# continental/uncertainty-detection-autolabeling

Measured on AMD Instinct MI355X. Metric: images*MC-samples/sec, EfficientDet-D0 MC-dropout serve (preprocess+net xT+decode+NMS), higher is better.
Workload: dtype f32 (tensors and accumulators float32; 1x1 products on the matrix cores as two fp16 pieces per operand, 3 cross terms (~2^-22 per product; float32-class, the default))

## Files before the change

### include/uda_hip.h

```cpp
#ifndef UDA_HIP_H_
#define UDA_HIP_H_

#include <stdint.h>

#ifdef __cplusplus
extern "C" {
#endif

#define UDA_ABI_VERSION 5
#define UDA_MAX_LEVELS 8
#define UDA_MAX_FUSE_INPUTS 3

typedef struct uda_buf_desc {
  int32_t H, W, C;
  int32_t per_sample;
  int64_t offset;
  int32_t kind;
  int32_t level;
} uda_buf_desc_t;

enum uda_op_kind {
  UDA_OP_STEM = 1,
  UDA_OP_PW = 2,
  UDA_OP_DW = 3,
  UDA_OP_SE = 4,
  UDA_OP_FUSE = 5,
  UDA_OP_POOL = 6,
  UDA_OP_MBX = 7,
  UDA_OP_SEP = 8
};
enum uda_act { UDA_ACT_NONE = 0, UDA_ACT_SWISH = 1, UDA_ACT_RELU = 2, UDA_ACT_RELU6 = 3, UDA_ACT_HSWISH = 4, UDA_ACT_MISH = 5 };
enum uda_resample { UDA_RS_NONE = 0, UDA_RS_NEAREST_UP = 1, UDA_RS_MAXPOOL = 2 };

typedef struct uda_op {
  int32_t kind;
  int32_t in[UDA_MAX_FUSE_INPUTS];
  int32_t out;
  int32_t se_scale;
  int32_t se_partial;
  int32_t residual;
  int32_t k, stride;
  int32_t act;
  int64_t w_off;
  int64_t bias_off;
  int64_t bn_scale_off;
  int64_t bn_shift_off;
  int64_t se_w1_off, se_b1_off, se_w2_off, se_b2_off;
  int32_t se_mid;
  int32_t drop_site;
  int32_t resample[UDA_MAX_FUSE_INPUTS];
  float fuse_w[UDA_MAX_FUSE_INPUTS];
  int32_t n_in;
  int32_t drop_site2;
  int64_t w2_off;
  int64_t bn2_scale_off, bn2_shift_off;
  int32_t launch_group;
  int32_t fuse_in;
  int32_t fuse_act;
} uda_op_t;

typedef struct uda_drop_site {
  int32_t channels;
  float rate;
} uda_drop_site_t;

enum uda_decode { UDA_DECODE_PLAIN = 0, UDA_DECODE_LNORM = 1, UDA_DECODE_FALSEDEC = 2,
                  UDA_DECODE_SAMPLE = 3  };
enum uda_post_mode { UDA_POST_GLOBAL = 0, UDA_POST_PER_CLASS = 1 };
enum uda_pw_scheme {
  UDA_SPLIT_NONE = 0,
  UDA_SPLIT_BF16X2 = 2,
  UDA_SPLIT_BF16X3 = 3,
  UDA_SPLIT_F16X2 = 4,
  UDA_SPLIT_F16X1 = 5
};

typedef struct uda_model {
  int32_t abi_version;
  int32_t image_h, image_w;
  float mean_rgb[3], stddev_rgb[3];
  int32_t num_levels;
  int32_t level_h[UDA_MAX_LEVELS], level_w[UDA_MAX_LEVELS];
  int32_t anchors_per_loc;
  int32_t num_classes;
  int32_t loss_attenuation;
  int32_t mc_samples;
  int32_t cls_stacked, box_stacked;
  int32_t has_uncert;
  int32_t decode_method;
  int32_t enable_softmax;
  float nms_soft_sigma;
  float nms_iou_thresh, nms_score_thresh;
  int32_t max_output_size;
  int32_t max_nms_inputs;
  int32_t post_mode;
  int32_t chunk_images;
  int32_t max_images;
  int64_t arena_floats;
  int32_t n_drop_sites;
  int32_t decode_nsamples;
  int32_t pw_scheme;
} uda_model_t;

typedef struct uda_ctx uda_ctx_t;

int uda_create(const uda_model_t* model, const uda_buf_desc_t* bufs, int32_t n_bufs,
               const uda_op_t* ops, int32_t n_ops, const uda_drop_site_t* sites,
               const float* weights, int64_t n_weights, const float* anchors ,
               int32_t device, uda_ctx_t** out);
void uda_destroy(uda_ctx_t* ctx);
const char* uda_last_error(const uda_ctx_t* ctx);

uint32_t uda_crc32c(const void* data, uint64_t n, uint32_t crc);

int uda_set_images_u8(uda_ctx_t* ctx, const uint8_t* images, int32_t n, int32_t h, int32_t w);
int uda_set_images_u8_ragged(uda_ctx_t* ctx, const uint8_t* const* images, int32_t n, const int32_t* h, const int32_t* w);
int uda_prefetch_images_u8(uda_ctx_t* ctx, const uint8_t* images, int32_t n, int32_t h, int32_t w);
int uda_prefetch_images_u8_ragged(uda_ctx_t* ctx, const uint8_t* const* images, int32_t n, const int32_t* h, const int32_t* w);
int uda_swap_prefetched(uda_ctx_t* ctx);
int uda_set_images_u8_device(uda_ctx_t* ctx, const void* images_dev, int32_t n, int32_t h, int32_t w);
int uda_input_u8_device(uda_ctx_t* ctx, const void** images_dev, int32_t* n, int32_t* h, int32_t* w);
int uda_set_images_f32(uda_ctx_t* ctx, const float* images, int32_t n, const float* image_scales);

int uda_set_dropout_seed(uda_ctx_t* ctx, uint64_t seed);
int uda_set_dropout_image_offset(uda_ctx_t* ctx, int64_t first_image);
int uda_set_dropout_sample_shard(uda_ctx_t* ctx, int32_t t_first, int32_t t_stride, int32_t t_total);
int uda_set_dropout_masks(uda_ctx_t* ctx, const float* masks, int64_t n_floats);
int uda_get_dropout_masks(uda_ctx_t* ctx, float* masks, int64_t n_floats);

int uda_run(uda_ctx_t* ctx, int32_t post_mode, int32_t run_post);
int uda_synchronize(uda_ctx_t* ctx);
int uda_run_async(uda_ctx_t* ctx, int32_t post_mode, int32_t* ticket);
int uda_run_consistency(uda_ctx_t* ctx, int32_t post_mode);
int uda_get_consistency(uda_ctx_t* ctx, double* iou, uint8_t* agree);
int uda_get_augmented_u8(uda_ctx_t* ctx, uint8_t* out, int64_t n_bytes);
int uda_collect(uda_ctx_t* ctx, int32_t ticket, float* boxes, float* scores, float* classes, int32_t* valid, float* logits);
int uda_collect_device(uda_ctx_t* ctx, int32_t ticket, int32_t rows, int32_t with_logits, void** dev_ptr, int32_t* cols);
int uda_drain(uda_ctx_t* ctx);
int64_t uda_range_demotions(const uda_ctx_t* ctx);
int uda_debug_op_scheme(const uda_ctx_t* ctx, int32_t op, int32_t* scheme, float* w_scale, float* a_scale, int32_t* out_f16);
int64_t uda_nms_prefix_fallbacks(const uda_ctx_t* ctx);
// ... 194 lines not shown
```

### uncertainty-detection-autolabeling_amd/capi.py

```python
import ctypes as C
import os
import subprocess

HERE = os.path.dirname(os.path.abspath(__file__))
CSRC = os.path.join(HERE, "csrc")
LIB_PATH = os.environ.get("UDA_LIB") or os.path.join(CSRC, "libuda_hip.so")
HEADER = os.path.join(os.path.dirname(HERE), "include", "uda_hip.h")

UDA_ABI_VERSION = 5
MAX_LEVELS = 8
MAX_FUSE = 3

OP_STEM, OP_PW, OP_DW, OP_SE, OP_FUSE, OP_POOL, OP_MBX, OP_SEP = 1, 2, 3, 4, 5, 6, 7, 8
ACT_NONE, ACT_SWISH, ACT_RELU, ACT_RELU6, ACT_HSWISH, ACT_MISH = 0, 1, 2, 3, 4, 5
RS_NONE, RS_NEAREST_UP, RS_MAXPOOL = 0, 1, 2
DECODE_PLAIN, DECODE_LNORM, DECODE_FALSEDEC, DECODE_SAMPLE = 0, 1, 2, 3
POST_GLOBAL, POST_PER_CLASS = 0, 1
CALIB_TS_ALL, CALIB_TS_PERCOO, CALIB_ISO_ALL, CALIB_ISO_PERCOO, CALIB_ISO_PERCLSCOO = 0, 1, 2, 3, 4
CLS_TS, CLS_ISO_ALL, CLS_ISO_PERCLS = 0, 1, 2
ASSIGN_IOU, ASSIGN_MSE, ASSIGN_RANK = 0, 1, 2
ASSIGN_KEEP_VALIDATE, ASSIGN_KEEP_CALIBRATE = 0, 1
SCORE_ENTROPY, SCORE_DET_SCORE, SCORE_ALBOX, SCORE_MCBOX, SCORE_MCCLASS = 0, 1, 2, 3, 4
SCORE_SCALAR, SCORE_MEAN, SCORE_REL_MEAN = 0, 1, 2
SCORE_MAX_COMP = 3
PROF_AGGREGATE, PROF_NMS, PROF_PREPROCESS, PROF_SCORE, PROF_EVAL, PROF_PSEUDO = 16, 17, 18, 19, 20, 21
EVAL_MAX_GT, EVAL_MAX_THRS = 256, 32
THR_MAX_N, THR_MAX_U, THR_MAX_THRS, THR_MAX_P, THR_MAX_G = 262144, 4, 32, 65536, 8192
PRUNE_ROWS, PRUNE_COLS, PRUNE_MAX_N, PRUNE_MAX_W = 256, 512, 1048576, 4
KNN_ROWS, KNN_COLS, KNN_MAX_D, KNN_MAX_N, KNN_MAX_B, KNN_MAX_PAIRS = 256, 512, 4, 1048576, 4096, 1 << 38
LC_MD, LC_MISTAKES, LC_NOISY = 1, 2, 4
LC_MD_EQ, LC_MD_LE = 0, 1
LC_GT_MISTAKE, LC_GT_NOISY, LC_GT_REPLACED = 1, 2, 4
LC_DET_KEPT, LC_DET_MISSING = 1, 2
LC_MAX_M, LC_MAX_G = 4096, 16384
AUDIT_DET_EXTRA, AUDIT_GT_NOMATCH = 1, 1
AUDIT_MAX_G, AUDIT_MAX_D, AUDIT_MAX_B = 1024, 1024, 1048576


class BufDesc(C.Structure):
    _fields_ = [("H", C.c_int32), ("W", C.c_int32), ("C", C.c_int32), ("per_sample", C.c_int32),
                ("offset", C.c_int64), ("kind", C.c_int32), ("level", C.c_int32)]


class Op(C.Structure):
    _fields_ = [("kind", C.c_int32), ("in_", C.c_int32 * MAX_FUSE), ("out", C.c_int32),
                ("se_scale", C.c_int32), ("se_partial", C.c_int32), ("residual", C.c_int32),
                ("k", C.c_int32), ("stride", C.c_int32), ("act", C.c_int32),
                ("w_off", C.c_int64), ("bias_off", C.c_int64), ("bn_scale_off", C.c_int64),
                ("bn_shift_off", C.c_int64), ("se_w1_off", C.c_int64), ("se_b1_off", C.c_int64),
                ("se_w2_off", C.c_int64), ("se_b2_off", C.c_int64), ("se_mid", C.c_int32),
                ("drop_site", C.c_int32), ("resample", C.c_int32 * MAX_FUSE),
                ("fuse_w", C.c_float * MAX_FUSE), ("n_in", C.c_int32), ("drop_site2", C.c_int32),
                ("w2_off", C.c_int64), ("bn2_scale_off", C.c_int64), ("bn2_shift_off", C.c_int64),
                ("launch_group", C.c_int32), ("fuse_in", C.c_int32), ("fuse_act", C.c_int32)]


class DropSite(C.Structure):
    _fields_ = [("channels", C.c_int32), ("rate", C.c_float)]


class Model(C.Structure):
    _fields_ = [("abi_version", C.c_int32), ("image_h", C.c_int32), ("image_w", C.c_int32),
                ("mean_rgb", C.c_float * 3), ("stddev_rgb", C.c_float * 3),
                ("num_levels", C.c_int32), ("level_h", C.c_int32 * MAX_LEVELS),
                ("level_w", C.c_int32 * MAX_LEVELS), ("anchors_per_loc", C.c_int32),
                ("num_classes", C.c_int32), ("loss_attenuation", C.c_int32),
                ("mc_samples", C.c_int32), ("cls_stacked", C.c_int32), ("box_stacked", C.c_int32),
                ("has_uncert", C.c_int32), ("decode_method", C.c_int32),
                ("enable_softmax", C.c_int32), ("nms_soft_sigma", C.c_float),
                ("nms_iou_thresh", C.c_float), ("nms_score_thresh", C.c_float),
                ("max_output_size", C.c_int32), ("max_nms_inputs", C.c_int32),
                ("post_mode", C.c_int32), ("chunk_images", C.c_int32), ("max_images", C.c_int32),
                ("arena_floats", C.c_int64), ("n_drop_sites", C.c_int32), ("decode_nsamples", C.c_int32),
                ("pw_scheme", C.c_int32)]


class ScoreTerm(C.Structure):
    _fields_ = [("source", C.c_int32), ("transform", C.c_int32), ("weight", C.c_double)]


class ScoreDesc(C.Structure):
    _fields_ = [("n_comp", C.c_int32), ("reduce_mean", C.c_int32), ("n_terms", C.c_int32 * SCORE_MAX_COMP),
                ("reserved", C.c_int32), ("term", (ScoreTerm * 2) * SCORE_MAX_COMP)]


_P = C.c_void_p
_SIGNATURES = {
    "uda_create": (C.c_int, [C.POINTER(Model), C.POINTER(BufDesc), C.c_int32, C.POINTER(Op), C.c_int32,
                             C.POINTER(DropSite), _P, C.c_int64, _P, C.c_int32, C.POINTER(_P)]),
    "uda_destroy": (None, [_P]),
    "uda_last_error": (C.c_char_p, [_P]),
    "uda_set_images_u8": (C.c_int, [_P, _P, C.c_int32, C.c_int32, C.c_int32]),
    "uda_set_images_u8_device": (C.c_int, [_P, _P, C.c_int32, C.c_int32, C.c_int32]),
    "uda_set_images_u8_ragged": (C.c_int, [_P, _P, C.c_int32, _P, _P]),
    "uda_input_u8_device": (C.c_int, [_P, C.POINTER(_P), C.POINTER(C.c_int32), C.POINTER(C.c_int32), C.POINTER(C.c_int32)]),
    "uda_prefetch_images_u8": (C.c_int, [_P, _P, C.c_int32, C.c_int32, C.c_int32]),
    "uda_prefetch_images_u8_ragged": (C.c_int, [_P, _P, C.c_int32, _P, _P]),
    "uda_swap_prefetched": (C.c_int, [_P]),
    "uda_set_images_f32": (C.c_int, [_P, _P, C.c_int32, _P]),
    "uda_set_dropout_seed": (C.c_int, [_P, C.c_uint64]),
    "uda_set_dropout_image_offset": (C.c_int, [_P, C.c_int64]),
    "uda_set_dropout_sample_shard": (C.c_int, [_P, C.c_int32, C.c_int32, C.c_int32]),
    "uda_set_dropout_masks": (C.c_int, [_P, _P, C.c_int64]),
    "uda_get_dropout_masks": (C.c_int, [_P, _P, C.c_int64]),
    "uda_run": (C.c_int, [_P, C.c_int32, C.c_int32]),
    "uda_synchronize": (C.c_int, [_P]),
    "uda_run_async": (C.c_int, [_P, C.c_int32, C.POINTER(C.c_int32)]),
    "uda_run_consistency": (C.c_int, [_P, C.c_int32]),
    "uda_get_consistency": (C.c_int, [_P, _P, _P]),
    "uda_get_augmented_u8": (C.c_int, [_P, _P, C.c_int64]),
    "uda_collect": (C.c_int, [_P, C.c_int32, _P, _P, _P, _P, _P]),
    "uda_collect_device": (C.c_int, [_P, C.c_int32, C.c_int32, C.c_int32, C.POINTER(_P), C.POINTER(C.c_int32)]),
    "uda_drain": (C.c_int, [_P]),
    "uda_range_demotions": (C.c_int64, [_P]),
    "uda_debug_op_scheme": (C.c_int, [_P, C.c_int32, C.POINTER(C.c_int32), C.POINTER(C.c_float), C.POINTER(C.c_float),
                                      C.POINTER(C.c_int32)]),
    "uda_nms_prefix_fallbacks": (C.c_int64, [_P]),
    "uda_nms_coop_fallbacks": (C.c_int64, [_P]),
    "uda_nms_coop_not_launched": (C.c_int64, [_P]),
    "uda_get_detections": (C.c_int, [_P, _P, _P, _P, _P, _P]),
    "uda_detection_cols": (C.c_int, [_P, C.c_int32, C.POINTER(C.c_int32), C.POINTER(C.c_int32)]),
    "uda_detections_device": (C.c_int, [_P, C.c_int32, C.c_int32, C.POINTER(_P), C.POINTER(C.c_int32)]),
    "uda_get_class_probs": (C.c_int, [_P, _P, _P]),
    "uda_set_ground_truth": (C.c_int, [_P, _P, _P, C.c_int32, C.c_int32]),
    "uda_assign_ground_truth": (C.c_int, [_P, C.c_int32, C.c_int32]),
    "uda_get_assignment": (C.c_int, [_P, _P, _P, _P]),
    "uda_get_assigned_rows": (C.c_int, [_P, _P, C.c_int64]),
    "uda_assigned_row_cols": (C.c_int, [_P, C.POINTER(C.c_int32)]),
    "uda_assign_gt_np": (C.c_int, [C.c_int32, _P, _P, _P, C.c_int32, C.c_int32, C.c_int32, C.c_int32, C.c_int32, _P, _P, _P]),
    "uda_score_images": (C.c_int, [_P, C.POINTER(ScoreDesc), C.c_float]),
    "uda_image_scores_shape": (C.c_int, [_P, C.POINTER(C.c_int32), C.POINTER(C.c_int32)]),
    "uda_get_image_scores": (C.c_int, [_P, _P, _P, _P]),
    "uda_score_images_np": (C.c_int, [C.c_int32, C.POINTER(ScoreDesc), C.c_double, _P, _P, _P, _P, _P, _P, _P, C.c_int32, C.c_int32,
                                      C.c_int32, C.c_int32, _P, _P, _P]),
    "uda_score_images_np_f32": (C.c_int, [C.c_int32, C.POINTER(ScoreDesc), C.c_float, _P, _P, _P, _P, _P, _P, _P, C.c_int32, C.c_int32,
                                          C.c_int32, C.c_int32, _P, _P, _P]),
    "uda_pseudo_rows": (C.c_int, [_P, C.POINTER(ScoreDesc), C.c_int32, C.c_int32, C.c_float, C.c_double, C.c_int32]),
# ... 86 lines not shown
```

### uncertainty-detection-autolabeling_amd/csrc/kernels_pwb.hip

```cpp
#include <math.h>
#include <stdio.h>
#include <stdlib.h>
#include <string.h>

#include <type_traits>

#include "mfma_common.h"

namespace uda {

template <int MT, int NT, int WM, int WN, int PARTS, int OCC, bool DEEP = false>
__global__ __launch_bounds__(256, OCC) void pwb_kernel(PwArgs a) {
  static_assert(WM * WN == 4, "four waves per block");
  constexpr int NPC = split_np(PARTS);
  constexpr int BM = 32 * MT * WM, NTB = NT * WN, BN = 32 * NTB;
  constexpr int A_BYTES = NPC * BM * PWB_AROW;
  constexpr int B_BYTES = 2 * NTB * NPC * 1024;
  constexpr int STG_BYTES = 4 * 32 * PWB_STG * 4;
  constexpr int LDS_BYTES = (A_BYTES + B_BYTES) > STG_BYTES ? (A_BYTES + B_BYTES) : STG_BYTES;
  __shared__ __attribute__((aligned(16))) unsigned char lds[LDS_BYTES];
  unsigned char* As = lds;
  uint4* Bs = (uint4*)(lds + A_BYTES);

  const int tid = threadIdx.x, lane = tid & 63, wave = tid >> 6;
  const int li = lane & 31, lh = lane >> 5;
  const int wr = wave / WN, wc = wave % WN;
  const int bx = blockIdx.x, by = blockIdx.y;
  const int b = blockIdx.z, b_in = b / a.in_div;
  const int m0 = bx * BM, n0 = by * BN;
  const int nt0 = by * NTB;
  const float* A = a.in + (size_t)b_in * a.HW * a.Cin;
  const bool in_h = PARTS == UDA_SPLIT_F16X1 && a.in_f16;
  const unsigned short* Ah = (const unsigned short*)a.in + (size_t)b_in * a.HW * a.Cin;
  const float* se = a.se ? a.se + (size_t)(b / a.se_div) * a.Cin : nullptr;
  const uint4* Wp = (const uint4*)a.wsplit;
  const int KS = (a.Cin + 15) >> 4;
  const int NTL = (a.Cout + 31) >> 5;

  f32x16 acc[MT][NT];
#pragma unroll
  for (int m = 0; m < MT; ++m)
#pragma unroll
    for (int n = 0; n < NT; ++n)
#pragma unroll
      for (int r = 0; r < 16; ++r) acc[m][n][r] = 0.f;

  constexpr int A_ITERS = BM * 8 / 256;
  constexpr int B_TOTAL = 2 * NTB * NPC * 64;
  constexpr int B_ITERS = (B_TOTAL + 255) / 256;
  struct ChunkRegs { float4 ra[A_ITERS]; uint4 rb[B_ITERS]; float4 rg; };
  ChunkRegs c0, c1;
  c0.rg = make_float4(1.f, 1.f, 1.f, 1.f);
  c1.rg = c0.rg;
  float amax = 0.f;

  auto load_chunk = [&](int k0, ChunkRegs& cr) {
    float4* ra = cr.ra; uint4* rb = cr.rb; float4& rg = cr.rg;
#pragma unroll
    for (int i = 0; i < A_ITERS; ++i) {
      const int f = tid + 256 * i;
      const int m = f >> 3, k = k0 + 4 * (f & 7);
      if constexpr (DEEP) {
        const int mr = m0 + m < a.HW ? m0 + m : a.HW - 1;
        ra[i] = *(const float4*)(A + (size_t)mr * a.Cin + k);
      } else if (in_h) {
        uint2 h = make_uint2(0u, 0u);
        if (m0 + m < a.HW && k < a.Cin) h = *(const uint2*)(Ah + (size_t)(m0 + m) * a.Cin + k);
        ra[i] = make_float4(__uint_as_float(h.x), __uint_as_float(h.y), 0.f, 0.f);
      } else {
        float4 v = make_float4(0.f, 0.f, 0.f, 0.f);
        if (m0 + m < a.HW && k < a.Cin) v = *(const float4*)(A + (size_t)(m0 + m) * a.Cin + k);
        ra[i] = v;
      }
    }
    if (se) {
      const int k = k0 + 4 * (tid & 7);
      if constexpr (DEEP) rg = *(const float4*)(se + k);
      else rg = (k < a.Cin) ? *(const float4*)(se + k) : make_float4(1.f, 1.f, 1.f, 1.f);
    }
    const int ks0 = k0 >> 4;
#pragma unroll
    for (int i = 0; i < B_ITERS; ++i) {
      const int f = tid + 256 * i;
      int q = f >> 6;
      const int part = q % NPC; q /= NPC;
      const int nt = q % NTB, ks = q / NTB;
      if constexpr (DEEP && B_TOTAL % 256 == 0) {
        rb[i] = Wp[(((size_t)(ks0 + ks) * NTL + (nt0 + nt)) * NPC + part) * 64 + (f & 63)];
      } else {
        uint4 v = make_uint4(0u, 0u, 0u, 0u);
        if (f < B_TOTAL && ks0 + ks < KS && nt0 + nt < NTL)
          v = Wp[(((size_t)(ks0 + ks) * NTL + (nt0 + nt)) * NPC + part) * 64 + (f & 63)];
        rb[i] = v;
      }
    }
  };
  auto store_chunk = [&](const ChunkRegs& cr) {
    const float4* ra = cr.ra; const uint4* rb = cr.rb; const float4 rg = cr.rg;
#pragma unroll
    for (int i = 0; i < A_ITERS; ++i) {
      const int f = tid + 256 * i;
      const int m = f >> 3, kq = f & 7;
      const float4 av = (!DEEP && in_h) ? f16x4_to_float4(__float_as_uint(ra[i].x), __float_as_uint(ra[i].y)) : ra[i];
      float r0 = av.x * rg.x, r1 = av.y * rg.y, r2 = av.z * rg.z, r3 = av.w * rg.w;
      split_track<PARTS>(amax, r0, r1);
      split_track<PARTS>(amax, r2, r3);
#pragma unroll
      for (int p = 0; p < NPC; ++p) {
        const unsigned u0 = pack_piece<PARTS>(r0, r1), u1 = pack_piece<PARTS>(r2, r3);
        *(uint2*)(As + (size_t)(p * BM + m) * PWB_AROW + kq * 8) = make_uint2(u0, u1);
        if (p + 1 < NPC) {
// ... 71 lines not shown
        if (col >= a.Cout) continue;
        const float bias = a.bias ? a.bias[col] : 0.f;
        const float sc = a.bn_scale ? a.bn_scale[col] : 1.f;
        const float sh = a.bn_scale ? a.bn_shift[col] : 0.f;
        const float mk = a.mask ? a.mask[(size_t)b * a.Cout + col] : 1.f;
#pragma unroll
        for (int r = 0; r < 16; ++r) {
          const int m = m0 + (wr * MT + m_) * 32 + (r & 3) + 8 * (r >> 2) + 4 * lh;
          if (m >= a.HW) continue;
          float v = fmaf(acc[m_][n][r], un, bias);
          v = fmaf(v, sc, sh);
          if (a.act == UDA_ACT_SWISH) v = swishf_b(v);
          else if (a.act >= UDA_ACT_RELU) v = act_relu_family(v, a.act);
          v *= mk;
          if (a.res) v += a.res[(res_base + m) * a.Cout + col];
          a.out[(out_base + m) * a.Cout + col] = v;
        }
      }
    return;
  }

  float* stg = (float*)lds + wave * 32 * PWB_STG;
  const int rrow = lane >> 4, c4 = lane & 15;
#pragma unroll
  for (int m_ = 0; m_ < MT; ++m_) {
#pragma unroll
    for (int p = 0; p < (NT + 1) / 2; ++p) {
#pragma unroll
      for (int q = 0; q < 2; ++q) {
        const int n = 2 * p + q;
        if (n < NT) {
#pragma unroll
          for (int r = 0; r < 16; ++r) stg[((r & 3) + 8 * (r >> 2) + 4 * lh) * PWB_STG + q * 32 + li] = acc[m_][n][r];
        }
      }
      __syncthreads();
      const int lcol = (wc * NT + 2 * p) * 32 + 4 * c4;
      const int col = n0 + lcol;
      const bool colok = (col < a.Cout) && (2 * p * 32 + 4 * c4 < NT * 32);
      const int colc = colok ? col : 0;
      float4 bias = make_float4(0.f, 0.f, 0.f, 0.f), sc = make_float4(1.f, 1.f, 1.f, 1.f);
      float4 sh = make_float4(0.f, 0.f, 0.f, 0.f), mk = make_float4(1.f, 1.f, 1.f, 1.f);
      if (a.bias) bias = *(const float4*)(a.bias + colc);
      if (a.bn_scale) {
        sc = *(const float4*)(a.bn_scale + colc);
        sh = *(const float4*)(a.bn_shift + colc);
      }
      if (a.mask) mk = *(const float4*)(a.mask + (size_t)b * a.Cout + colc);
      const int mrow0 = m0 + (wr * MT + m_) * 32 + rrow;
      float4 rr[8], v[8];
      if (a.res) {
#pragma unroll
        for (int it = 0; it < 8; ++it) {
          const int mc = mrow0 + it * 4 < a.HW ? mrow0 + it * 4 : a.HW - 1;
          rr[it] = *(const float4*)(a.res + (res_base + mc) * a.Cout + colc);
        }
      }
#pragma unroll
      for (int it = 0; it < 8; ++it) v[it] = *(const float4*)(stg + (it * 4 + rrow) * PWB_STG + 4 * c4);
#pragma unroll
      for (int it = 0; it < 8; ++it) {
        float4 t = v[it];
        t.x = fmaf(fmaf(t.x, un, bias.x), sc.x, sh.x);
        t.y = fmaf(fmaf(t.y, un, bias.y), sc.y, sh.y);
        t.z = fmaf(fmaf(t.z, un, bias.z), sc.z, sh.z);
        t.w = fmaf(fmaf(t.w, un, bias.w), sc.w, sh.w);
        if (a.act == UDA_ACT_SWISH) {
          t.x = swishf_b(t.x); t.y = swishf_b(t.y); t.z = swishf_b(t.z); t.w = swishf_b(t.w);
        } else if (a.act >= UDA_ACT_RELU) {
          t.x = act_relu_family(t.x, a.act); t.y = act_relu_family(t.y, a.act); t.z = act_relu_family(t.z, a.act); t.w = act_relu_family(t.w, a.act);
        }
        t.x *= mk.x; t.y *= mk.y; t.z *= mk.z; t.w *= mk.w;
        if (a.res) { t.x += rr[it].x; t.y += rr[it].y; t.z += rr[it].z; t.w += rr[it].w; }
        v[it] = t;
      }
#pragma unroll
      for (int it = 0; it < 8; ++it) {
        const int m = mrow0 + it * 4;
        if (colok && m < a.HW) *(float4*)(a.out + (out_base + m) * a.Cout + col) = v[it];
      }
      __syncthreads();
    }
  }
}

__global__ __launch_bounds__(256, 3) void pwb_shared_kernel(PwArgs a) {
  constexpr int WAVE_BYTES = 32 * PWB_STG * 4;
  __shared__ __attribute__((aligned(16))) unsigned char lds[4 * WAVE_BYTES];
  const int tid = threadIdx.x, lane = tid & 63, wave = tid >> 6;
  const int li = lane & 31, lh = lane >> 5;
  unsigned char* Aw = lds + wave * WAVE_BYTES;
  float* stg = (float*)Aw;
  const int b_in = blockIdx.z;
  const int m0 = blockIdx.x * 128 + wave * 32;
  const float* A = a.in + (size_t)b_in * a.HW * a.Cin;
  const uint4* Wp = (const uint4*)a.wsplit;
  const int NTL = (a.Cout + 31) >> 5;
  float4 ra[4];
#pragma unroll
  for (int i = 0; i < 4; ++i) {
    const int m = (lane >> 3) + 8 * i, k = 4 * (lane & 7);
    ra[i] = (m0 + m < a.HW && k < a.Cin) ? *(const float4*)(A + (size_t)(m0 + m) * a.Cin + k) : make_float4(0.f, 0.f, 0.f, 0.f);
  }
  bf16x8 bf[2][2];
  const int KS = (a.Cin + 15) >> 4;
#pragma unroll
  for (int ks = 0; ks < 2; ++ks)
#pragma unroll
    for (int p = 0; p < 2; ++p)
      bf[ks][p] = __builtin_bit_cast(bf16x8, ks < KS ? Wp[(((size_t)ks * NTL) * 2 + p) * 64 + lane] : make_uint4(0u, 0u, 0u, 0u));
  const int rrow = lane >> 4, c4 = lane & 15;
  const int col = 4 * c4;
  const bool colok = col < a.Cout;
  float4 bias = make_float4(0.f, 0.f, 0.f, 0.f), sc = make_float4(1.f, 1.f, 1.f, 1.f), sh = make_float4(0.f, 0.f, 0.f, 0.f);
  if (colok && (a.Cout & 3) == 0) {
    if (a.bias) bias = *(const float4*)(a.bias + col);
    if (a.bn_scale) { sc = *(const float4*)(a.bn_scale + col); sh = *(const float4*)(a.bn_shift + col); }
  }

  for (int t = 0; t < a.in_div; ++t) {
    const int b = b_in * a.in_div + t;
    float4 rg = make_float4(1.f, 1.f, 1.f, 1.f);
    if (a.se) {
      const int k = 4 * (lane & 7);
      if (k < a.Cin) rg = *(const float4*)(a.se + (size_t)(b / a.se_div) * a.Cin + k);
    }
#pragma unroll
    for (int i = 0; i < 4; ++i) {
      const int m = (lane >> 3) + 8 * i, kq = lane & 7;
      float r0 = ra[i].x * rg.x, r1 = ra[i].y * rg.y, r2 = ra[i].z * rg.z, r3 = ra[i].w * rg.w;
#pragma unroll
      for (int p = 0; p < 2; ++p) {
        const unsigned u0 = pack_bf16(r0, r1), u1 = pack_bf16(r2, r3);
        *(uint2*)(Aw + (size_t)(p * 32 + m) * PWB_AROW + kq * 8) = make_uint2(u0, u1);
        if (p == 0) {
          r0 -= bf16_lo_f32(u0); r1 -= bf16_hi_f32(u0);
          r2 -= bf16_lo_f32(u1); r3 -= bf16_hi_f32(u1);
        }
      }
    }
    __builtin_amdgcn_wave_barrier();
    f32x16 acc;
#pragma unroll
    for (int r = 0; r < 16; ++r) acc[r] = 0.f;
#pragma unroll
    for (int ks = 0; ks < 2; ++ks) {
      const bf16x8 a0 = *(const bf16x8*)(Aw + (size_t)(0 * 32 + li) * PWB_AROW + ks * 32 + lh * 16);
      const bf16x8 a1 = *(const bf16x8*)(Aw + (size_t)(1 * 32 + li) * PWB_AROW + ks * 32 + lh * 16);
      acc = __builtin_amdgcn_mfma_f32_32x32x16_bf16(a1, bf[ks][0], acc, 0, 0, 0);
      acc = __builtin_amdgcn_mfma_f32_32x32x16_bf16(a0, bf[ks][1], acc, 0, 0, 0);
      acc = __builtin_amdgcn_mfma_f32_32x32x16_bf16(a0, bf[ks][0], acc, 0, 0, 0);
    }
    __builtin_amdgcn_wave_barrier();
#pragma unroll
    for (int r = 0; r < 16; ++r) stg[((r & 3) + 8 * (r >> 2) + 4 * lh) * PWB_STG + li] = acc[r];
    __builtin_amdgcn_wave_barrier();
    float4 mk = make_float4(1.f, 1.f, 1.f, 1.f);
    if (colok && a.mask) mk = *(const float4*)(a.mask + (size_t)b * a.Cout + col);
    const size_t out_base = (size_t)b * a.HW;
    const size_t res_base = a.res ? (size_t)(b / a.res_div) * a.HW : 0;
#pragma unroll
    for (int it = 0; it < 8; ++it) {
      const int row = it * 4 + rrow;
      const int m = m0 + row;
      if (colok && m < a.HW) {
        float4 v = *(const float4*)(stg + row * PWB_STG + col);
// ... 170 lines not shown
    if constexpr (MT * NT > 4) {
      if (a.Cin >= 384 && a.Cin % PWB_BK == 0 && a.Cout % BN == 0 && (2 * NT * WN * 2 * 64) % 256 == 0) { hipLaunchKernelGGL((pwb_kernel<MT, NT, WM, WN, 4, 2, true>), grid, block, 0, s, a); return; }
    }
    hipLaunchKernelGGL((pwb_kernel<MT, NT, WM, WN, 4, (MT * NT > 4 ? 2 : 3)>), grid, block, 0, s, a);
  }
  else hipLaunchKernelGGL((pwb_kernel<MT, NT, WM, WN, 2, (MT * NT > 4 ? 2 : 3)>), grid, block, 0, s, a);
}

void launch_pwb(const PwArgs& a, int rows, hipStream_t s) {
  static const int shared = uda_env_int("UDA_PW_SHARED", 1);
  if (shared && a.in_div > 1 && a.Cin <= 32 && a.Cout <= 32 && (a.Cout & 3) == 0 && a.wparts == 2 && rows % a.in_div == 0) {
    const dim3 grid((a.HW + 127) / 128, 1, rows / a.in_div);
    hipLaunchKernelGGL(pwb_shared_kernel, grid, dim3(256), 0, s, a);
    return;
  }
  if (launch_pws(a, rows, s)) return;
  int cfg = a.Cout <= 32 ? 1 : (a.Cout <= 64 ? 2 : (a.Cout <= 96 ? 3 : 4));
  if (a.Cout > 128) {
    const int bn[3] = {128, 160, 192}, id[3] = {4, 6, 5};
    int best = 1 << 30;
    for (int i = 0; i < 3; ++i) {
      const int waste = (a.Cout + bn[i] - 1) / bn[i] * bn[i] - a.Cout;
      if (waste <= best) { best = waste; cfg = id[i]; }
    }
  }
  switch (cfg) {
    case 1: launch_pwb_cfg<1, 1, 4, 1>(a, rows, s); break;
    case 2: launch_pwb_cfg<1, 2, 4, 1>(a, rows, s); break;
    case 3: launch_pwb_cfg<1, 3, 4, 1>(a, rows, s); break;
    case 5: launch_pwb_cfg<2, 3, 2, 2>(a, rows, s); break;
    case 6: launch_pwb_cfg<1, 5, 4, 1>(a, rows, s); break;
    default: launch_pwb_cfg<2, 2, 2, 2>(a, rows, s); break;
  }
}

#ifndef UDA_MBX_ET
#define UDA_MBX_ET 3
#endif
__host__ __device__ constexpr int mbx_et_w(int k, int s) {
  return s != 1 ? 0 : (k == 5 ? ((UDA_MBX_ET & 1) ? 4 : 0) : ((UDA_MBX_ET & 2) ? 2 : 0));
}
__host__ __device__ constexpr int mbx_et_pitch(int w) { return w == 2 ? 258 : 260; }
template <int W>
__device__ __forceinline__ void et_store_slice(float* ep, const f32x16& acc) {
#pragma unroll
  for (int q = 0; q < 4; ++q) {
    const float v0 = swish_core(acc[4 * q]), v1 = swish_core(acc[4 * q + 1]), v2 = swish_core(acc[4 * q + 2]), v3 = swish_core(acc[4 * q + 3]);
    if constexpr (W == 4) {
      *(float4*)(ep + 8 * q) = make_float4(v0, v1, v2, v3);
    } else {
      *(float2*)(ep + 8 * q) = make_float2(v0, v1);
      *(float2*)(ep + 8 * q + 2) = make_float2(v2, v3);
    }
  }
}
template <int W>
__device__ __forceinline__ void et_read(float* dst, const float* er, int jj) {
  if constexpr (W == 4) {
    const float4 v = *(const float4*)(er + 4 * jj);
    dst[4 * jj] = v.x; dst[4 * jj + 1] = v.y; dst[4 * jj + 2] = v.z; dst[4 * jj + 3] = v.w;
  } else {
    const float2 v = *(const float2*)(er + 2 * jj);
    dst[2 * jj] = v.x; dst[2 * jj + 1] = v.y;
  }
}

namespace {
struct MbxCfgB { int th, tw; };
__host__ __device__ constexpr MbxCfgB mbxb_cfg(int k, int s) {
  return s == 1 ? (k == 3 ? MbxCfgB{12, 16} : MbxCfgB{8, 16}) : (k == 3 ? MbxCfgB{7, 8} : MbxCfgB{4, 10});
}
}

#ifndef UDA_MBXB_WK_LDS
#define UDA_MBXB_WK_LDS 1
#endif
#ifndef UDA_MBXB6_W
#define UDA_MBXB6_W 3
#endif
#ifndef UDA_MBXB_MINW
#define UDA_MBXB_MINW(K, S, KSF, PARTS) ((PARTS) == 3 ? (((KSF) <= 2 && (K) == 3) ? UDA_MBXB6_W : 2) : \
    ((KSF) <= 2 ? ((K) == 3 ? 4 : 3) : (((KSF) <= 3 && ((K) == 3 ? (S) == 2 : UDA_MBXB_WK_LDS)) ? 3 : 2)))
#endif
template <int K, int S, int KSF, bool FUSE0, int PARTS, bool OH = false>
__global__ __launch_bounds__(256, UDA_MBXB_MINW(K, S, KSF, PARTS)) void mbxb_kernel(MbxArgs a) {
  constexpr int NW = 4;
  constexpr int NPC = split_np(PARTS);
  constexpr int TH = mbxb_cfg(K, S).th, TW = mbxb_cfg(K, S).tw;
  constexpr int IH = (TH - 1) * S + K, IW = (TW - 1) * S + K;
  constexpr int NP = IH * IW;
  constexpr int NPP = (NP + 31) / 32 * 32;
  constexpr int NMT = NPP / 32;
  constexpr int NG = NW * 2;
  constexpr int MTW = (NMT + NW - 1) / NW;
  constexpr int ES = 32;
  constexpr int ETW = mbx_et_w(K, S);
  constexpr bool ET = ETW != 0;
  constexpr int CP = mbx_et_pitch(ETW);
  constexpr int XW = (S == 1) ? 8 : (K == 3 ? (TW == 8 ? 8 : 6) : 5);
  constexpr int UPR = TW / XW;
  constexpr int NUNIT = TH * UPR;
  static_assert(TW % XW == 0, "units must tile the output tile");
  constexpr int NCOL = (XW - 1) * S + K;
  extern __shared__ __attribute__((aligned(16))) float mlds[];
  float* E = mlds;
  float* red = E + (ET ? (size_t)32 * CP : (size_t)NPP * ES);
  constexpr int NPAR = (K * K + 2) * 32;
  float* par = red + NG * 32;
  constexpr bool B_LDS = KSF <= 2;
  constexpr int BSLAB = KSF * NPC * 64;
  uint4* Bs = (uint4*)(par + 2 * NPAR);

  const int tid = threadIdx.x, lane = tid & 63, wave = tid >> 6;
  const int li = lane & 31, lh = lane >> 5;
  int tbx = blockIdx.x, tby = blockIdx.y, b = blockIdx.z;
  if (a.remap_T > 0) {
    const int T = a.remap_T, nt = a.tiles_x * a.tiles_y, ntp = (nt + 7) & ~7;
    const unsigned L = blockIdx.x;
    const unsigned per_img = (unsigned)ntp * (unsigned)T;
    const int img = (int)(L / per_img);
    const unsigned r = L - (unsigned)img * per_img;
    const int grp = (int)(r / (8u * (unsigned)T)), w = (int)(r % (8u * (unsigned)T));
    const int tl = grp * 8 + (w & 7);
    if (tl >= nt) return;
    b = img * T + (w >> 3);
    tby = tl / a.tiles_x;
    tbx = tl - tby * a.tiles_x;
  }
  const int b_in = b / a.in_div;
  const int oy0 = tby * TH, ox0 = tbx * TW;
  const int iy0 = oy0 * S - a.pad_t, ix0 = ox0 * S - a.pad_l;
  const int cin_mem = FUSE0 ? a.c0 : a.Cin;
  const float* xin = a.in + (size_t)b_in * a.H * a.W * cin_mem;

  float amax = 0.f;
  bf16x8 w0p[2][NPC];
  float sh0v[8];
  if constexpr (FUSE0) {
    if (a.w0frag) {
      const uint4* fp = a.w0frag + (size_t)(b / a.g_div) * (2 * NPC * 64) + lane;
#pragma unroll
      for (int ks = 0; ks < 2; ++ks)
#pragma unroll
        for (int p_ = 0; p_ < NPC; ++p_) w0p[ks][p_] = __builtin_bit_cast(bf16x8, fp[(ks * NPC + p_) * 64]);
    } else {
      const float* gp = a.gate + (size_t)(b / a.g_div) * a.c0;
#pragma unroll
      for (int ks = 0; ks < 2; ++ks) {
        const int k = ks * 16 + 8 * lh;
        float4 w0 = *(const float4*)(a.w0t + li * 32 + k), w1 = *(const float4*)(a.w0t + li * 32 + k + 4);
        const float4 g0 = *(const float4*)(gp + k), g1 = *(const float4*)(gp + k + 4);
        w0.x *= g0.x; w0.y *= g0.y; w0.z *= g0.z; w0.w *= g0.w;
        w1.x *= g1.x; w1.y *= g1.y; w1.z *= g1.z; w1.w *= g1.w;
        split_parts<PARTS>(w0, w1, w0p[ks], amax);
      }
    }
#pragma unroll
    for (int j = 0; j < 8; ++j) sh0v[j] = a.sh0f[(j & 3) + 8 * (j >> 2) + 4 * lh];
  }

  bf16x8 ap[MTW][KSF][NPC];
#pragma unroll
  for (int t = 0; t < MTW; ++t) {
    const int mt = wave + NW * t;
    const int p = mt * 32 + li;
    const int iy = iy0 + p / IW, ix = ix0 + p % IW;
    const bool in = (mt < NMT) && (p < NP) && iy >= 0 && iy < a.H && ix >= 0 && ix < a.W;
    const float* px = xin + ((size_t)(in ? iy : 0) * a.W + (in ? ix : 0)) * cin_mem;
    if constexpr (FUSE0) {
      static_assert(!FUSE0 || KSF == 2, "the fused projection feeds a 16-channel expand");
      f32x16 xacc;
#pragma unroll
      for (int r = 0; r < 16; ++r) xacc[r] = 0.f;
#pragma unroll
      for (int ks = 0; ks < 2; ++ks) {
        const int k = ks * 16 + 8 * lh;
        float4 d0 = make_float4(0.f, 0.f, 0.f, 0.f), d1 = d0;
        if (in) {
          d0 = *(const float4*)(px + k);
          d1 = *(const float4*)(px + k + 4);
        }
        bf16x8 dp[NPC];
        split_parts<PARTS>(d0, d1, dp, amax);
        xacc = mfma_terms<PARTS>(w0p[ks], dp, xacc);
      }
      float4 v0, v1;
      v0.x = in ? xacc[0] + sh0v[0] : 0.f; v0.y = in ? xacc[1] + sh0v[1] : 0.f;
      v0.z = in ? xacc[2] + sh0v[2] : 0.f; v0.w = in ? xacc[3] + sh0v[3] : 0.f;
      v1.x = in ? xacc[4] + sh0v[4] : 0.f; v1.y = in ? xacc[5] + sh0v[5] : 0.f;
      v1.z = in ? xacc[6] + sh0v[6] : 0.f; v1.w = in ? xacc[7] + sh0v[7] : 0.f;
      split_parts<PARTS>(v0, v1, ap[t][0], amax);
      float4 f0 = make_float4((lh == 0 && in) ? 1.f : 0.f, 0.f, 0.f, 0.f), f1 = make_float4(0.f, 0.f, 0.f, 0.f);
      split_parts<PARTS>(f0, f1, ap[t][1]);
      continue;
    }
#pragma unroll
    for (int ks = 0; ks < KSF; ++ks) {
      const int k = ks * 16 + 8 * lh;
      float4 v0 = make_float4(0.f, 0.f, 0.f, 0.f), v1 = v0;
      if (in && k < a.Cin) {
        v0 = *(const float4*)(px + k);
// ... 127 lines not shown
      for (int i = 0; i < P_PER; ++i) {
        const int f = tid + 256 * i;
        if (more && f < NPAR) pnext[f] = np_[i];
      }
      asm volatile("" : "+v"(mk0n), "+v"(mk1n));
    }
    constexpr bool WK_LDS = UDA_MBXB_WK_LDS && K == 5 && KSF == 3;
    float wk[WK_LDS ? 1 : K * K];
    if constexpr (!WK_LDS) {
#pragma unroll
      for (int t = 0; t < K * K; ++t) wk[t] = pcur[t * 32 + c];
    }
    const float sc1 = pcur[K * K * 32 + c] * mk0, sh1 = pcur[(K * K + 1) * 32 + c];
    float ssum = 0.f;
    float* const ob = obase + ch * 32;
    unsigned short* const hob = hobase + ch * 32;
    auto dw_units = [&](auto guard) {
      constexpr bool GUARD = decltype(guard)::value;
      constexpr int KYU = (UDA_MBXB_WK_LDS && K == 5 && KSF == 3) ? 1 : K;
#pragma unroll
      for (int ui = 0; ui < UPT; ++ui) {
        if constexpr (UNIT_GUARD) {
          if (g + NG * ui >= NUNIT) continue;
        }
        if constexpr (GUARD) {
          if (oy0 + (g + NG * ui) / UPR >= a.Ho) continue;
        }
        float acc[XW];
#pragma unroll
        for (int o = 0; o < XW; ++o) acc[o] = 0.f;
        const float* eu = E + eoff[ui];
#pragma unroll KYU
        for (int ky = 0; ky < K; ++ky) {
          float rowv[NCOL];
          if constexpr (ET) {
            static_assert(!ET || NCOL % ETW == 0, "whole 16- / 8-byte reads");
#pragma unroll
            for (int jj = 0; jj < NCOL / (ET ? ETW : 1); ++jj) et_read<ETW>(rowv, eu + ky * IW, jj);
          } else {
#pragma unroll
            for (int j = 0; j < NCOL; ++j) rowv[j] = eu[(ky * IW + j) * ES];
          }
#pragma unroll
          for (int kx = 0; kx < K; ++kx) {
            const float w = WK_LDS ? pcur[(ky * K + kx) * 32 + c] : wk[WK_LDS ? 0 : ky * K + kx];
#pragma unroll
            for (int o = 0; o < XW; ++o) acc[o] = fmaf(rowv[o * S + kx], w, acc[o]);
          }
        }
#pragma unroll
        for (int o = 0; o < XW; ++o) {
          bool ok = true;
          if constexpr (GUARD) ok = ox0 + (int)((g + NG * ui) % UPR) * XW + o < a.Wo;
          if (ok) {
            const float v = swish_folded(fmaf(acc[o], sc1, sh1), mk1);
            if constexpr (OH) store_uniform_base_h(hob + (size_t)o * cm, ooff[ui], v);
            else store_uniform_base(ob + (size_t)o * cm, ooff[ui], v);
            ssum += v;
          }
        }
        __builtin_amdgcn_sched_barrier(0);
      }
    };
    if (dcol) {
      if (full) dw_units(std::false_type());
      else dw_units(std::true_type());
    }
    if (a.se_partial) red[g * 32 + c] = ssum;
    __syncthreads();
    if (a.se_partial && g == 0 && dcol) {
      float t = red[c];
#pragma unroll
      for (int gg = 1; gg < NG; ++gg) t += red[gg * 32 + c];
      a.se_partial[((size_t)b * a.n_tiles + tile) * a.Cmid + col] = t;
    }
    mk0 = mk0n;
    mk1 = mk1n;
    if constexpr (!B_LDS) {
#pragma unroll
      for (int ks = 0; ks < KR; ++ks)
#pragma unroll
        for (int p_ = 0; p_ < NPC; ++p_) rb[ks][p_] = nbr[ks][p_];
    }
  }
}

template <int PARTS>
__global__ __launch_bounds__(64) void w0gate_kernel(const float* gate, const float* w0t, int c0, uint4* out, unsigned* oor) {
  constexpr int NPC = split_np(PARTS);
  const int row = blockIdx.x, lane = threadIdx.x, li = lane & 31, lh = lane >> 5;
  const float* gp = gate + (size_t)row * c0;
  float amax = 0.f;
#pragma unroll
  for (int ks = 0; ks < 2; ++ks) {
    const int k = ks * 16 + 8 * lh;
    float4 w0 = *(const float4*)(w0t + li * 32 + k), w1 = *(const float4*)(w0t + li * 32 + k + 4);
    const float4 g0 = *(const float4*)(gp + k), g1 = *(const float4*)(gp + k + 4);
    w0.x *= g0.x; w0.y *= g0.y; w0.z *= g0.z; w0.w *= g0.w;
    w1.x *= g1.x; w1.y *= g1.y; w1.z *= g1.z; w1.w *= g1.w;
    bf16x8 pc[NPC];
    split_parts<PARTS>(w0, w1, pc, amax);
#pragma unroll
    for (int p_ = 0; p_ < NPC; ++p_) out[((size_t)row * 2 * NPC + ks * NPC + p_) * 64 + lane] = __builtin_bit_cast(uint4, pc[p_]);
  }
  split_report<PARTS>(amax, oor);
}

size_t mbxb_w0frag_elems(int gate_rows, int scheme) { return (size_t)gate_rows * 2 * uda_split_pieces(scheme) * 64; }
void launch_w0gate(const float* gate, const float* w0t, int c0, int gate_rows, int scheme, uint4* out, unsigned* oor, hipStream_t s) {
  if (scheme == UDA_SPLIT_BF16X3) hipLaunchKernelGGL(w0gate_kernel<3>, dim3(gate_rows), dim3(64), 0, s, gate, w0t, c0, out, oor);
  else if (scheme == UDA_SPLIT_F16X2) hipLaunchKernelGGL(w0gate_kernel<4>, dim3(gate_rows), dim3(64), 0, s, gate, w0t, c0, out, oor);
  else if (scheme == UDA_SPLIT_F16X1) hipLaunchKernelGGL(w0gate_kernel<5>, dim3(gate_rows), dim3(64), 0, s, gate, w0t, c0, out, oor);
  else hipLaunchKernelGGL(w0gate_kernel<2>, dim3(gate_rows), dim3(64), 0, s, gate, w0t, c0, out, oor);
}

int mbxb_tiles(int Ho, int Wo, int k, int stride) {
  const MbxCfgB c = mbxb_cfg(k, stride);
  return ((Ho + c.th - 1) / c.th) * ((Wo + c.tw - 1) / c.tw);
}

bool mbxb_supported(int Cin, int Cmid, int k, int stride) {
  return Cin % 8 == 0 && Cin >= 16 && Cin <= 48 && Cmid % 4 == 0 && (k == 3 || k == 5) && (stride == 1 || stride == 2);
}

template <int K, int S, int KSF, int PARTS>
static void launch_mbxb_t(const MbxArgs& a, int rows, hipStream_t s) {
  constexpr int TH = mbxb_cfg(K, S).th, TW = mbxb_cfg(K, S).tw;
  constexpr int IH = (TH - 1) * S + K, IW = (TW - 1) * S + K;
  constexpr int NPP = (IH * IW + 31) / 32 * 32;
  const size_t lds = ((mbx_et_w(K, S) ? (size_t)32 * mbx_et_pitch(mbx_et_w(K, S)) : (size_t)NPP * 32) + 8 * 32 + 2 * (K * K + 2) * 32) * sizeof(float) +
                     (size_t)KSF * split_np(PARTS) * 64 * sizeof(uint4);
  dim3 grid((a.Wo + TW - 1) / TW, (a.Ho + TH - 1) / TH, rows);
  MbxArgs b = a;
  b.remap_T = 0;
  if (a.in_div > 1 && rows % a.in_div == 0) {
    const long long nt = (long long)grid.x * grid.y, ntp = (nt + 7) / 8 * 8;
    const long long total = ntp * rows;
    if (total < (1ll << 31)) {
      b.remap_T = a.in_div; b.tiles_x = (int)grid.x; b.tiles_y = (int)grid.y;
      grid = dim3((unsigned)total, 1, 1);
    }
  }
  if constexpr (PARTS == UDA_SPLIT_F16X1) {
    if (a.out_f16) {
      if constexpr (KSF == 2) {
        if (a.gate) { hipLaunchKernelGGL((mbxb_kernel<K, S, KSF, true, PARTS, true>), grid, dim3(256), lds, s, b); return; }
      }
      hipLaunchKernelGGL((mbxb_kernel<K, S, KSF, false, PARTS, true>), grid, dim3(256), lds, s, b);
      return;
    }
  }
  if constexpr (KSF == 2) {
    if (a.gate) { hipLaunchKernelGGL((mbxb_kernel<K, S, KSF, true, PARTS>), grid, dim3(256), lds, s, b); return; }
  }
  hipLaunchKernelGGL((mbxb_kernel<K, S, KSF, false, PARTS>), grid, dim3(256), lds, s, b);
}

template <int K, int S, int PARTS>
static void launch_mbxb_ks(const MbxArgs& a, int rows, hipStream_t s) {
  switch ((a.Cin + 1 + 15) / 16) {
    case 2: launch_mbxb_t<K, S, 2, PARTS>(a, rows, s); break;
    case 3: launch_mbxb_t<K, S, 3, PARTS>(a, rows, s); break;
    default: launch_mbxb_t<K, S, 4, PARTS>(a, rows, s); break;
  }
}

template <int PARTS>
static void launch_mbxb_p(const MbxArgs& a, int rows, int k, int stride, hipStream_t s) {
  if (k == 3 && stride == 1) launch_mbxb_ks<3, 1, PARTS>(a, rows, s);
  else if (k == 3 && stride == 2) launch_mbxb_ks<3, 2, PARTS>(a, rows, s);
  else if (k == 5 && stride == 1) launch_mbxb_ks<5, 1, PARTS>(a, rows, s);
  else launch_mbxb_ks<5, 2, PARTS>(a, rows, s);
}

void launch_mbxb(const MbxArgs& a, int rows, int k, int stride, hipStream_t s) {
  if (a.wparts == UDA_SPLIT_BF16X3) launch_mbxb_p<3>(a, rows, k, stride, s);
  else if (a.wparts == UDA_SPLIT_F16X2) launch_mbxb_p<4>(a, rows, k, stride, s);
  else if (a.wparts == UDA_SPLIT_F16X1) launch_mbxb_p<5>(a, rows, k, stride, s);
  else launch_mbxb_p<2>(a, rows, k, stride, s);
}

struct MbxCfgD { int th, tw, xw; };
__host__ __device__ constexpr MbxCfgD mbxd_cfg(int k, int s, bool wide = false) {
  return s == 1 ? (wide ? (k == 3 ? MbxCfgD{8, 20, 10} : MbxCfgD{6, 20, 4}) : (k == 3 ? MbxCfgD{12, 16, 4} : MbxCfgD{8, 16, 8}))
                : (k == 3 ? MbxCfgD{7, 8, 8} : MbxCfgD{4, 10, 5});
}
__host__ __device__ constexpr long long mbxd_slots(int Ho, int Wo, int k, bool wide) {
  return (long long)((Ho + mbxd_cfg(k, 1, wide).th - 1) / mbxd_cfg(k, 1, wide).th) * mbxd_cfg(k, 1, wide).th *
         ((Wo + mbxd_cfg(k, 1, wide).tw - 1) / mbxd_cfg(k, 1, wide).tw) * mbxd_cfg(k, 1, wide).tw;
}
bool mbxd_wide(int Ho, int Wo, int k, int stride) {
  return stride == 1 && mbxd_slots(Ho, Wo, k, true) < mbxd_slots(Ho, Wo, k, false);
}

__host__ __device__ constexpr bool mbxd_two_per_cu(int ksf, int parts, int s) { return (ksf <= 8 && parts != 3) || (parts == UDA_SPLIT_F16X1 && s == 1); }
template <int K, int KSF, int PARTS, int S, bool WIDE, bool OH = false>
__global__ __launch_bounds__(512, mbxd_two_per_cu(KSF, PARTS, S) ? 4 : 2) void mbxd_kernel(MbxArgs a) {
  constexpr bool WK_LDS = (K == 5 && (KSF <= 8 || PARTS == 3 || PARTS == UDA_SPLIT_F16X1));

  constexpr int NW = 8;
  constexpr int NPC = split_np(PARTS);
  static_assert(!WIDE || S == 1, "wide tiles are a stride-1 variant");
  constexpr int TH = mbxd_cfg(K, S, WIDE).th, TW = mbxd_cfg(K, S, WIDE).tw;
  constexpr int IH = (TH - 1) * S + K, IW = (TW - 1) * S + K;
  constexpr int NP = IH * IW;
  static_assert(NP <= 256, "input tile must fit 8 slices of 32 pixels");
  constexpr int NPP = 256;
  constexpr int NG = NW * 2;
  constexpr int ES = 33;
  constexpr int ETW = mbx_et_w(K, S);
  constexpr bool ET = ETW != 0;
  constexpr int CP = mbx_et_pitch(ETW);
  static_assert(!ET || (IW % ETW == 0 && mbxd_cfg(K, S, WIDE).xw % ETW == 0), "aligned wide accesses of the transposed slab");
  constexpr int XW = mbxd_cfg(K, S, WIDE).xw;
  constexpr int UPR = TW / XW;
  constexpr int NUNIT = TH * UPR;
  static_assert(TW % XW == 0, "units must tile the output tile");
  constexpr int NCOL = (XW - 1) * S + K;
  constexpr int BSLAB = KSF * NPC * 64;
  extern __shared__ __attribute__((aligned(16))) float dlds[];
  float* E = dlds;
  float* red = E + (size_t)NPP * ES;
  constexpr int NPAR = (K * K + 2) * 32;
  float* par = red + NG * 32;
  uint4* Bs = (uint4*)(par + 2 * NPAR);
  float* mks = (float*)(Bs + BSLAB);

  const int tid = threadIdx.x, lane = tid & 63, wave = tid >> 6;
  const int li = lane & 31, lh = lane >> 5;
  const int b = blockIdx.z / a.ch_groups, b_in = b / a.in_div;
  const int oy0 = blockIdx.y * TH, ox0 = blockIdx.x * TW;
  const int iy0 = oy0 * S - a.pad_t, ix0 = ox0 * S - a.pad_l;
  const float* xin = a.in + (size_t)b_in * a.H * a.W * a.Cin;
  const int NCH = (a.Cmid + 31) >> 5;
  const int ch_per = (NCH + a.ch_groups - 1) / a.ch_groups;
  const int chb = (int)(blockIdx.z % a.ch_groups) * ch_per;
  const int che = chb + ch_per < NCH ? chb + ch_per : NCH;
  if (chb >= che) return;
  const uint4* Wp = (const uint4*)a.wsplit;
  for (int f = tid; f < BSLAB; f += 512) {
    const int ks = f / (NPC * 64), rest = f - ks * (NPC * 64);
    Bs[f] = Wp[(((size_t)ks * NCH + chb) * NPC + (rest >> 6)) * 64 + (rest & 63)];
  }
  for (int f = tid; f < NPAR; f += 512) par[f] = a.wpar[(size_t)chb * NPAR + f];
  for (int f = tid; f < 2 * 32 * NCH; f += 512) {
    const int which = f / (32 * NCH), col = f - which * 32 * NCH;
    const float* m = which ? a.mask1 : a.mask0;
    mks[f] = ((m && col < a.Cmid) ? m[(size_t)b * a.Cmid + col] : 1.f) * UDA_NEG_LN2;
  }

  bf16x8 ap[KSF][NPC];
  float amax = 0.f;
  {
    const int p = wave * 32 + li;
    const int iy = iy0 + p / IW, ix = ix0 + p % IW;
    const bool in = (p < NP) && iy >= 0 && iy < a.H && ix >= 0 && ix < a.W;
    const float* px = xin + ((size_t)(in ? iy : 0) * a.W + (in ? ix : 0)) * a.Cin;
#pragma unroll
    for (int ks = 0; ks < KSF; ++ks) {
      const int k = ks * 16 + 8 * lh;
      float4 v0 = make_float4(0.f, 0.f, 0.f, 0.f), v1 = v0;
      if (in && k < a.Cin) {
// ... 767 lines not shown
```

### uncertainty-detection-autolabeling_amd/csrc/uda_api.hip

```cpp
#include <stdarg.h>
#include <stdio.h>
#include <stdlib.h>
#include <string.h>

#include <algorithm>
#include <numeric>
#include <string>
#include <vector>

#include "uda_ctx.h"

static thread_local std::string g_create_error;

static void set_f16_storage(uda_ctx* c);

int fail(uda_ctx* c, const char* fmt, ...) {
  char buf[1024];
  va_list ap;
  va_start(ap, fmt);
  vsnprintf(buf, sizeof(buf), fmt, ap);
  va_end(ap);
  if (c) c->err = buf; else g_create_error = buf;
  return 1;
}
// ... 186 lines not shown
  if (model->n_drop_sites > 0 && sites) c->sites.assign(sites, sites + model->n_drop_sites);
  c->device = device;
  c->n_weights = n_weights;
#define CK(expr)                                                                                  \
  do {                                                                                            \
    hipError_t e_ = (expr);                                                                       \
    if (e_ != hipSuccess) {                                                                       \
      fail(nullptr, "%s failed: %s (%s:%d)", #expr, hipGetErrorString(e_), __FILE__, __LINE__);  \
      uda_destroy(c);                                                                             \
      return 1;                                                                                   \
    }                                                                                             \
  } while (0)
  CK(hipSetDevice(device));
  CK(hipStreamCreateWithFlags(&c->stream, hipStreamNonBlocking));

  const uda_model_t& m = c->model;
  const int T = m.mc_samples;
  for (int i = 0; i < n_ops; ++i) {
    const uda_op_t& o = ops[i];
    auto okbuf = [&](int id) { return id >= 0 && id < n_bufs; };
    if (!okbuf(o.out)) { fail(nullptr, "op %d: bad out buffer %d", i, o.out); uda_destroy(c); return 1; }
    for (int j = 0; j < o.n_in; ++j)
      if (!okbuf(o.in[j])) { fail(nullptr, "op %d: bad in[%d] buffer %d", i, j, o.in[j]); uda_destroy(c); return 1; }
    if (o.drop_site >= m.n_drop_sites || ((o.kind == UDA_OP_MBX || o.kind == UDA_OP_SEP) && o.drop_site2 >= m.n_drop_sites)) {
      fail(nullptr, "op %d: bad drop site %d", i, o.drop_site);
      uda_destroy(c);
      return 1;
    }
    if (o.drop_site >= 0 && c->sites[o.drop_site].channels != bufs[o.out].C) {
      fail(nullptr, "op %d: drop site %d has %d channels, output has %d", i, o.drop_site,
           c->sites[o.drop_site].channels, bufs[o.out].C);
      uda_destroy(c);
      return 1;
    }
    if (o.kind == UDA_OP_MBX && o.se_scale >= 0 &&
        (!okbuf(o.se_scale) || o.se_mid != 16 || bufs[o.in[0]].C > 32 || bufs[o.in[0]].C % 8 || bufs[o.se_scale].C != bufs[o.in[0]].C ||
         o.se_w1_off < 0 || o.se_b1_off < 0 || o.se_w2_off < 0)) {
      fail(nullptr, "op %d: fused projection needs a [rows, C0 <= 32] gate, a 16-channel projection and its kernel / BN offsets", i);
      uda_destroy(c);
      return 1;
    }
    if (o.act < UDA_ACT_NONE || o.act > UDA_ACT_MISH || o.fuse_act < UDA_ACT_NONE || o.fuse_act > UDA_ACT_MISH) {
      fail(nullptr, "op %d: unknown activation %d / %d", i, o.act, o.fuse_act);
      uda_destroy(c);
      return 1;
    }
    if (o.kind == UDA_OP_MBX && o.act != UDA_ACT_SWISH) {
      fail(nullptr, "op %d: the fused MBConv front half is a swish kernel (act %d)", i, o.act);
      uda_destroy(c);
      return 1;
    }
    if (o.kind == UDA_OP_SEP && o.drop_site2 >= 0) {
      const uda_buf_desc_t& ib = bufs[o.in[0]];
      const uda_buf_desc_t& ob = bufs[o.out];
      if (o.fuse_in || ib.per_sample || (!ob.per_sample && T > 1) || c->sites[o.drop_site2].channels != ib.C) {
        fail(nullptr, "op %d: a deferred input dropout site needs a plain separable conv with a per-image input of %d channels and a "
                      "per-sample output", i, c->sites[o.drop_site2].channels);
        uda_destroy(c);
        return 1;
      }
    }
    if (o.fuse_in && o.kind != UDA_OP_SEP) {
      fail(nullptr, "op %d: fuse_in is a separable-conv field (kind %d)", i, o.kind);
      uda_destroy(c);
      return 1;
    }
    if (o.kind == UDA_OP_SEP && (o.w_off < 0 || o.w2_off < 0 || !sep_supported(bufs[o.in[0]].C, bufs[o.out].C) ||
                                 (!o.fuse_in && (bufs[o.in[0]].H != bufs[o.out].H || bufs[o.in[0]].W != bufs[o.out].W)))) {
      fail(nullptr, "op %d: fused separable conv %d->%d unsupported (needs both kernels, C %% 8 == 0, 16 <= C <= 128, same size)",
           i, bufs[o.in[0]].C, bufs[o.out].C);
      uda_destroy(c);
      return 1;
    }
    const int64_t offs[] = {o.w_off, o.bias_off, o.bn_scale_off, o.bn_shift_off, o.se_w1_off, o.se_b1_off, o.se_w2_off, o.se_b2_off,
                            (o.kind == UDA_OP_MBX || o.kind == UDA_OP_SEP) ? o.w2_off : -1, o.kind == UDA_OP_MBX ? o.bn2_scale_off : -1,
                            o.kind == UDA_OP_MBX ? o.bn2_shift_off : -1};
    for (int64_t off : offs)
      if (off >= n_weights) { fail(nullptr, "op %d: weight offset %lld beyond blob (%lld)", i, (long long)off, (long long)n_weights); uda_destroy(c); return 1; }
    if ((o.kind == UDA_OP_PW || o.kind == UDA_OP_DW || o.kind == UDA_OP_MBX) && (bufs[o.in[0]].C % 4 || bufs[o.out].C % 1)) {
      fail(nullptr, "op %d: channel count %d not a multiple of 4", i, bufs[o.in[0]].C);
      uda_destroy(c);
      return 1;
    }
  }
  for (int i = 0; i < n_bufs; ++i) {
    const uda_buf_desc_t& b = bufs[i];
    if (b.kind == 0) {
      const int64_t rows = (int64_t)m.chunk_images * (b.per_sample ? T : 1);
      const int64_t end = b.offset + rows * b.H * b.W * b.C;
      if (b.offset < 0 || end > m.arena_floats) {
        fail(nullptr, "buffer %d [%dx%dx%d] exceeds the arena (%lld > %lld)", i, b.H, b.W, b.C,
             (long long)end, (long long)m.arena_floats);
        uda_destroy(c);
        return 1;
      }
    }
  }

  CK(dalloc(&c->d_weights, (size_t)n_weights));
  CK(hipMemcpy(c->d_weights, weights, (size_t)n_weights * sizeof(float), hipMemcpyHostToDevice));
  {
    c->pw_parts = m.pw_scheme;
    c->wsplit_off.assign(n_ops, -1);
    c->wpar_off.assign(n_ops, -1);
    c->wscheme.assign(n_ops, c->pw_parts);
    c->buf_f16.assign(n_bufs, 0);
    c->wunscale.assign(n_ops, 1.0f);
    c->wascale.assign(n_ops, 1.0f);
    CK(dalloc(&c->d_oor, 2 * ((size_t)n_ops + 1)));
    CK(hipMemset(c->d_oor, 0, 2 * ((size_t)n_ops + 1) * sizeof(unsigned)));
    c->oor_cur = c->d_oor;
    c->wovr.assign(n_ops, nullptr);
    c->wovr_par.assign(n_ops, -1);
    c->h_weights.assign(weights, weights + n_weights);
    if (c->pw_parts) {
      std::vector<uint16_t> packed;
      for (int i = 0; i < n_ops; ++i) {
        const uda_op_t& o = ops[i];
        if (o.w_off < 0) continue;
        const int K = bufs[o.in[0]].C, Nn = bufs[o.out].C;
        const size_t at = packed.size();
        if (o.kind == UDA_OP_PW || o.kind == UDA_OP_SEP) {
          float scale = 1.0f;
          const int sch = c->pw_parts;
          if (uda_split_f16(sch)) {
            scale = split_weight_scale(weights + o.w_off, (size_t)K * Nn);
            c->wunscale[i] = 1.0f / scale;
            ++c->n_f16_ops;
          }
          c->wscheme[i] = sch;
          const size_t w_elems = (pwb_packed_elems(K, Nn, sch) + 7) / 8 * 8;
          size_t dw_fl = 0;
          float ascale = 1.0f;
          if (o.kind == UDA_OP_SEP && uda_split_f16(sch) && o.w2_off >= 0) {
            constexpr int SEP_F16_TAP_SHIFT = 6;
            ascale = ldexpf(1.0f, SEP_F16_TAP_SHIFT);
            dw_fl = (size_t)9 * K;
          }
          packed.resize(at + w_elems + 2 * dw_fl);
          pwb_pack_weights(weights + o.w_off, K, Nn, sch, packed.data() + at, scale);
          if (dw_fl) {
            std::vector<float> wd(dw_fl);
            for (size_t j = 0; j < dw_fl; ++j) wd[j] = weights[o.w2_off + j] * ascale;
            memcpy(packed.data() + at + w_elems, wd.data(), dw_fl * sizeof(float));
            c->wpar_off[i] = (int64_t)(at + w_elems);
            c->wunscale[i] /= ascale;
            c->wascale[i] = ascale;
          }
        } else if (o.kind == UDA_OP_MBX && o.bn_scale_off >= 0 && o.bn_shift_off >= 0 &&
                   (mbxb_supported(o.se_scale >= 0 ? o.se_mid : K, Nn, o.k, o.stride) || mbxd_supported(K, Nn, o.k, o.stride))) {
          if (o.w2_off < 0 || o.bn2_scale_off < 0 || o.bn2_shift_off < 0) continue;
          const bool fuse0 = o.se_scale >= 0;
          const int Ke = fuse0 ? o.se_mid : K;
          int sch = c->pw_parts;
          if (uda_split_f16(sch)) {
            std::vector<uint16_t> probe(mbxb_packed_elems(Ke, Nn, sch));
            float st[2] = {0.f, 0.f};
            mbxb_pack_weights(weights + o.w_off, weights + o.bn_scale_off, weights + o.bn_shift_off, Ke, Nn, probe.data(), fuse0, sch, st);
            static const float min_rms = getenv("UDA_F16_MIN_RMS") ? (float)atof(getenv("UDA_F16_MIN_RMS")) : 0.015625f;
            const bool rms_ok = sch == UDA_SPLIT_F16X1 || st[1] >= min_rms;
            if (!(st[0] < 32768.0f) || !rms_ok) { sch = UDA_SPLIT_BF16X3; ++c->n_f16_demoted; }
            else ++c->n_f16_ops;
          }
          c->wscheme[i] = sch;
          const size_t we_elems = (mbxb_packed_elems(Ke, Nn, sch) + 7) / 8 * 8;
          const size_t par_fl = mbx_par_floats(Nn, o.k);
// ... 290 lines not shown
  const uda_ctx::U8Slot& sl = c->u8[c->cur];
  if (!c->have_u8 || !sl.valid) return fail(c, "input_u8_device: no uint8 batch is set");
  for (int i = 1; i < sl.n; ++i)
    if (sl.geo[i].h != sl.geo[0].h || sl.geo[i].w != sl.geo[0].w) return fail(c, "input_u8_device: the batch has several raw sizes");
  HIPC(c, hipEventSynchronize(sl.ev));
  *images_dev = sl.d_img; *n = sl.n; *h = sl.geo[0].h; *w = sl.geo[0].w;
  return 0;
}

extern "C" int uda_swap_prefetched(uda_ctx_t* c) {
  if (!c) return 1;
  if (!c->u8[c->cur ^ 1].valid) return fail(c, "swap_prefetched: nothing was prefetched");
  HIPC(c, hipSetDevice(c->device));
  c->u8[c->cur].valid = false;
  return make_current(c, c->cur ^ 1);
}

extern "C" int uda_set_images_f32(uda_ctx_t* c, const float* images, int32_t n, const float* image_scales) {
  if (!c || !images) return c ? fail(c, "set_images_f32: NULL images") : 1;
  if (n < 1 || n > c->model.max_images) return fail(c, "set_images_f32: n=%d outside [1, %d]", n, c->model.max_images);
  HIPC(c, hipSetDevice(c->device));
  const size_t fl = (size_t)n * c->model.image_h * c->model.image_w * 3;
  HIPC(c, hipMemcpyAsync(c->d_images, images, fl * sizeof(float), hipMemcpyHostToDevice, c->stream));
  for (int i = 0; i < n; ++i) c->h_scales[i] = image_scales ? image_scales[i] : 1.0f;
  HIPC(c, hipMemcpyAsync(c->d_scales, c->h_scales.data(), n * sizeof(float), hipMemcpyHostToDevice, c->stream));
  c->n_images = n;
  c->noise_from = -1;
  c->have_u8 = false;
  c->stem_from_u8 = false;
  ++c->f32_gen;
  return 0;
}

extern "C" int uda_set_dropout_seed(uda_ctx_t* c, uint64_t seed) {
  if (!c) return 1;
  c->seed = seed;
  c->masks_injected = false;
  return 0;
}

extern "C" int uda_set_dropout_image_offset(uda_ctx_t* c, int64_t first_image) {
  if (!c) return 1;
  if (first_image < 0) return fail(c, "set_dropout_image_offset: negative offset");
  c->image_offset = first_image;
  return 0;
}

extern "C" int uda_set_dropout_sample_shard(uda_ctx_t* c, int32_t t_first, int32_t t_stride, int32_t t_total) {
  if (!c) return 1;
  const int T = c->model.mc_samples;
  if (t_total == 0) { c->t_first = 0; c->t_stride = 1; c->t_total = 0; return 0; }
  if (t_first < 0 || t_stride < 1 || t_total < T || t_first + (int64_t)(T - 1) * t_stride >= t_total)
    return fail(c, "set_dropout_sample_shard: samples %d + j * %d (j < %d) do not lie inside %d", t_first, t_stride, T, t_total);
  c->t_first = t_first; c->t_stride = t_stride; c->t_total = t_total;
  return 0;
}

extern "C" int uda_set_dropout_masks(uda_ctx_t* c, const float* masks, int64_t n_floats) {
  if (!c || !masks) return c ? fail(c, "set_dropout_masks: NULL") : 1;
  if (n_floats > c->mask_cap || (c->sum_site_ch && n_floats % c->sum_site_ch))
    return fail(c, "set_dropout_masks: %lld floats is not rows*%lld (capacity %lld)", (long long)n_floats,
                (long long)c->sum_site_ch, (long long)c->mask_cap);
  HIPC(c, hipSetDevice(c->device));
  if (n_floats) HIPC(c, hipMemcpyAsync(c->d_masks, masks, n_floats * sizeof(float), hipMemcpyHostToDevice, c->stream));
  c->masks_injected = true;
  ++c->masks_gen;
  c->masks_rows = c->sum_site_ch ? (int)(n_floats / c->sum_site_ch) : 0;
  return 0;
}

extern "C" int uda_get_dropout_masks(uda_ctx_t* c, float* masks, int64_t n_floats) {
  if (!c || !masks) return 1;
  if (n_floats > c->mask_cap) return fail(c, "get_dropout_masks: too many floats");
  HIPC(c, hipSetDevice(c->device));
  HIPC(c, hipStreamSynchronize(c->stream));
  if (n_floats) HIPC(c, hipMemcpy(masks, c->d_masks, n_floats * sizeof(float), hipMemcpyDeviceToHost));
  return 0;
}

struct ChunkView {
  uda_ctx* c;
  int i0, nc;
  int lane = 0;
  hipStream_t stream() const { return c->lane_stream[lane]; }
  int rows(const uda_buf_desc_t& b) const { return nc * (b.per_sample ? c->model.mc_samples : 1); }
  float* ptr(int id) const {
    const uda_buf_desc_t& b = c->bufs[id];
    const size_t per = (size_t)b.H * b.W * b.C;
    const int T = c->model.mc_samples;
    switch (b.kind) {
      case 1: return c->d_images + (size_t)i0 * per;
      case 2: return c->d_cls[b.level] + (size_t)i0 * (b.per_sample ? T : 1) * per;
      case 3: return c->d_box[b.level] + (size_t)i0 * (b.per_sample ? T : 1) * per;
      default: return c->lane_arena[lane] + b.offset;
    }
  }
  const float* wt(int64_t off) const { return off < 0 ? nullptr : c->d_weights + off; }
  const float* mask(int site) const {
    if (site < 0) return nullptr;
    return c->d_masks + c->site_off[site] + (size_t)i0 * c->model.mc_samples * c->sites[site].channels;
  }
  int div(const uda_buf_desc_t& in, const uda_buf_desc_t& out) const {
    return (out.per_sample && !in.per_sample) ? c->model.mc_samples : 1;
  }
};

static inline const uint16_t* wsplit_of(const uda_ctx* c, int oi) { return c->wovr[oi] ? c->wovr[oi] : c->d_wsplit + c->wsplit_off[oi]; }
static inline bool has_wpar(const uda_ctx* c, int oi) { return c->wovr[oi] ? c->wovr_par[oi] >= 0 : c->wpar_off[oi] >= 0; }
static inline const uint16_t* wpar_of(const uda_ctx* c, int oi) {
  return c->wovr[oi] ? c->wovr[oi] + c->wovr_par[oi] : c->d_wsplit + c->wpar_off[oi];
}

static int fill_fuse_args(uda_ctx* c, const ChunkView& v, int oi, FuseArgs& a) {
  const uda_op_t& o = c->ops[oi];
  const uda_buf_desc_t& ob = c->bufs[o.out];
  a.n_in = o.n_in;
  a.H = ob.H; a.W = ob.W;
  if (o.n_in < 1 || o.n_in > UDA_MAX_FUSE_INPUTS) return fail(c, "op %d: %d fusion inputs", oi, o.n_in);
  a.C = c->bufs[o.in[0]].C;
  if (a.C % 4) return fail(c, "op %d: fuse needs channels %% 4 == 0", oi);
  for (int i = 0; i < o.n_in; ++i) {
    const uda_buf_desc_t& ib = c->bufs[o.in[i]];
    if (ib.C != a.C) return fail(c, "op %d: fuse input %d has %d channels, input 0 %d", oi, i, ib.C, a.C);
    a.in[i] = v.ptr(o.in[i]);
    a.wgt[i] = (o.kind == UDA_OP_POOL) ? 1.0f : o.fuse_w[i];
    a.mode[i] = o.resample[i];
    a.Hi[i] = ib.H; a.Wi[i] = ib.W;
    a.in_div[i] = v.div(ib, ob);
    if (a.mode[i] == UDA_RS_NONE) {
      if (ib.H != ob.H || ib.W != ob.W) return fail(c, "op %d: fuse input %d size mismatch", oi, i);
    } else if (a.mode[i] == UDA_RS_NEAREST_UP) {
      if (ib.H > ob.H || ib.W > ob.W) return fail(c, "op %d: nearest-up input %d larger than output", oi, i);
      a.sy[i] = (float)ib.H / (float)ob.H;
      a.sx[i] = (float)ib.W / (float)ob.W;
    } else if (a.mode[i] == UDA_RS_MAXPOOL) {
      const int sh_ = (ib.H - 1) / ob.H + 1, sw_ = (ib.W - 1) / ob.W + 1;
      if (sh_ != sw_) return fail(c, "op %d: non-square pooling window", oi);
      a.ps[i] = sh_;
      a.pk[i] = sh_ + 1;
      if ((ib.H + sh_ - 1) / sh_ != ob.H || (ib.W + sh_ - 1) / sh_ != ob.W)
        return fail(c, "op %d: pooled size mismatch", oi);
      a.ppt[i] = same_pad_before(ib.H, ob.H, a.pk[i], a.ps[i]);
      a.ppl[i] = same_pad_before(ib.W, ob.W, a.pk[i], a.ps[i]);
    } else {
      return fail(c, "op %d: unknown resample mode %d of input %d", oi, a.mode[i], i);
    }
  }
  return 0;
}

static int run_op(uda_ctx* c, const ChunkView& v, int oi) {
  const uda_op_t& o = c->ops[oi];
  const uda_buf_desc_t& ob = c->bufs[o.out];
  const int rows = v.rows(ob);
  ProfScope ps(c, o.kind, v.stream());
  switch (o.kind) {
    case UDA_OP_STEM: {
      const uda_buf_desc_t& ib = c->bufs[o.in[0]];
      if (ib.C != 3 || ob.C % 4) return fail(c, "op %d: stem needs 3 -> 4k channels", oi);
      if (ib.per_sample != ob.per_sample) return fail(c, "op %d: stem cannot change the sample axis", oi);
      StemArgs a{};
      a.in = v.ptr(o.in[0]);
      a.out = v.ptr(o.out);
      a.w = v.wt(o.w_off);
      a.bn_scale = v.wt(o.bn_scale_off);
      a.bn_shift = v.wt(o.bn_shift_off);
      a.H = ib.H; a.W = ib.W; a.Ho = ob.H; a.Wo = ob.W; a.Co = ob.C;
      a.pad_t = same_pad_before(ib.H, ob.H, 3, 2);
      a.pad_l = same_pad_before(ib.W, ob.W, 3, 2);
      a.rows = rows;
      a.act = o.act;
      if (c->stem_from_u8) {
        if (ib.kind != 1 || ib.per_sample) return fail(c, "op %d: the uint8 stem reads the image buffer", oi);
        const uda_ctx::U8Slot& sl = c->u8[c->cur];
        a.u8 = sl.d_img; a.geo = sl.d_geo; a.img0 = v.i0;
        for (int k = 0; k < 3; ++k) { a.mean[k] = c->model.mean_rgb[k]; a.stdv[k] = c->model.stddev_rgb[k]; }
      }
      launch_stem(a, v.stream());
      break;
    }
    case UDA_OP_PW: {
      const uda_buf_desc_t& ib = c->bufs[o.in[0]];
      if (ib.H != ob.H || ib.W != ob.W) return fail(c, "op %d: 1x1 conv changes the spatial size", oi);
      PwArgs a{};
      a.in = v.ptr(o.in[0]);
      a.out = v.ptr(o.out);
      a.w = v.wt(o.w_off);
      a.bias = v.wt(o.bias_off);
      a.bn_scale = v.wt(o.bn_scale_off);
      a.bn_shift = v.wt(o.bn_shift_off);
      a.se = o.se_scale >= 0 ? v.ptr(o.se_scale) : nullptr;
      a.in_f16 = c->buf_f16[o.in[0]];
      a.se_div = 1;
      if (o.se_scale >= 0) {
        const uda_buf_desc_t& sb = c->bufs[o.se_scale];
        if (sb.per_sample && !ob.per_sample) return fail(c, "op %d: per-sample SE gate on a per-image output", oi);
        if (!sb.per_sample && ib.per_sample) return fail(c, "op %d: per-image SE gate on a per-sample input", oi);
        a.se_div = v.div(sb, ob);
      }
      a.mask = v.mask(o.drop_site);
      a.res = o.residual >= 0 ? v.ptr(o.residual) : nullptr;
      a.HW = ob.H * ob.W; a.Cin = ib.C; a.Cout = ob.C;
      a.in_div = v.div(ib, ob);
      a.res_div = o.residual >= 0 ? v.div(c->bufs[o.residual], ob) : 1;
      a.act = o.act;
      if (c->wsplit_off[oi] >= 0) {
        a.wsplit = wsplit_of(c, oi);
        a.wparts = c->wscheme[oi];
        a.wunscale = c->wunscale[oi];
        a.oor = c->oor_cur + oi;
        if (uda_split_f16(a.wparts)) c->oor_armed = true;
        launch_pwb(a, rows, v.stream());
      } else {
        launch_pw(a, rows, v.stream());
      }
      break;
    }
    case UDA_OP_DW: {
      const uda_buf_desc_t& ib = c->bufs[o.in[0]];
      if (ib.C != ob.C) return fail(c, "op %d: depthwise changes channels", oi);
      if (!((o.k == 3 || o.k == 5) && (o.stride == 1 || o.stride == 2)))
        return fail(c, "op %d: depthwise k=%d s=%d unsupported", oi, o.k, o.stride);
      DwArgs a{};
      a.in = v.ptr(o.in[0]);
      a.out = v.ptr(o.out);
      a.w = v.wt(o.w_off);
      a.bn_scale = v.wt(o.bn_scale_off);
      a.bn_shift = v.wt(o.bn_shift_off);
      a.mask = v.mask(o.drop_site);
      a.H = ib.H; a.W = ib.W; a.Ho = ob.H; a.Wo = ob.W; a.C = ob.C;
      a.pad_t = same_pad_before(ib.H, ob.H, o.k, o.stride);
      a.pad_l = same_pad_before(ib.W, ob.W, o.k, o.stride);
      a.in_div = v.div(ib, ob);
      a.act = o.act;
      if (o.se_partial >= 0) {
        const int nt = dw_tiles(ob.C, ob.H, ob.W, o.k, o.stride);
        const uda_buf_desc_t& pb = c->bufs[o.se_partial];
        if ((int64_t)pb.H * pb.W != (int64_t)nt || pb.C != ob.C || pb.per_sample != ob.per_sample)
          return fail(c, "op %d: SE partial buffer [%d,%d,%d] does not match %d tiles", oi, pb.H, pb.W, pb.C, nt);
        a.se_partial = v.ptr(o.se_partial);
      }
      launch_dw(a, rows, o.k, o.stride, v.stream());
      break;
    }
    case UDA_OP_MBX: {
      const uda_buf_desc_t& ib = c->bufs[o.in[0]];
      const bool fuse0 = o.se_scale >= 0;
      const int cin = fuse0 ? o.se_mid : ib.C;
      const bool deep = cin > 48;
      if (fuse0 && c->wsplit_off[oi] < 0) return fail(c, "op %d: the fused projection needs the split-bf16 path", oi);
      if (deep ? !(mbxd_supported(cin, ob.C, o.k, o.stride) && c->wsplit_off[oi] >= 0) : !mbx_supported(cin, ob.C, o.k, o.stride))
        return fail(c, "op %d: fused MBConv %d->%d k%d s%d unsupported", oi, cin, ob.C, o.k, o.stride);
      if (o.drop_site2 >= c->model.n_drop_sites || (o.drop_site2 >= 0 && c->sites[o.drop_site2].channels != ob.C))
        return fail(c, "op %d: bad second dropout site", oi);
      MbxArgs a{};
      a.in = v.ptr(o.in[0]);
      a.out = v.ptr(o.out);
      a.we = v.wt(o.w_off); a.sc0 = v.wt(o.bn_scale_off); a.sh0 = v.wt(o.bn_shift_off);
      a.wd = v.wt(o.w2_off); a.sc1 = v.wt(o.bn2_scale_off); a.sh1 = v.wt(o.bn2_shift_off);
      if (!a.we || !a.sc0 || !a.wd || !a.sc1) return fail(c, "op %d: fused MBConv needs both kernels and both BNs", oi);
      a.mask0 = v.mask(o.drop_site);
      a.mask1 = v.mask(o.drop_site2);
      a.H = ib.H; a.W = ib.W; a.Ho = ob.H; a.Wo = ob.W; a.Cin = cin; a.Cmid = ob.C;
      a.pad_t = same_pad_before(ib.H, ob.H, o.k, o.stride);
      a.pad_l = same_pad_before(ib.W, ob.W, o.k, o.stride);
      a.in_div = v.div(ib, ob);
      a.n_tiles = deep ? mbxd_tiles(ob.H, ob.W, o.k, o.stride)
                       : (c->wsplit_off[oi] >= 0 ? mbxb_tiles(ob.H, ob.W, o.k, o.stride) : mbx_tiles(ob.H, ob.W, o.k, o.stride));
      if (o.se_partial >= 0) {
        const uda_buf_desc_t& pb = c->bufs[o.se_partial];
        if ((int64_t)pb.H * pb.W != (int64_t)a.n_tiles || pb.C != ob.C || pb.per_sample != ob.per_sample)
          return fail(c, "op %d: SE partial buffer [%d,%d,%d] does not match %d tiles", oi, pb.H, pb.W, pb.C, a.n_tiles);
        a.se_partial = v.ptr(o.se_partial);
      }
      if (c->wsplit_off[oi] >= 0) {
        a.wsplit = wsplit_of(c, oi);
        a.wparts = c->wscheme[oi];
        a.oor = c->oor_cur + oi;
        if (uda_split_f16(a.wparts)) c->oor_armed = true;
        a.wpar = (const float*)wpar_of(c, oi);
        a.out_f16 = c->buf_f16[o.out];
        if (fuse0) {
          const uda_buf_desc_t& gb = c->bufs[o.se_scale];
          if (gb.per_sample && !ob.per_sample) return fail(c, "op %d: per-sample gate on a per-image output", oi);
          a.gate = v.ptr(o.se_scale);
          a.g_div = v.div(gb, ob);
          a.c0 = ib.C;
          a.w0t = a.wpar + mbx_par_floats(ob.C, o.k);
          a.sh0f = a.w0t + 32 * 32;
          if (ib.C == 32) {
            const int gate_rows = v.rows(gb);
            const int ln = v.lane & 1;
            const size_t need = mbxb_w0frag_elems(gate_rows, a.wparts);
            if (need > c->w0frag_cap[ln]) {
              HIPC(c, hipStreamSynchronize(v.stream()));
              if (c->d_w0frag[ln]) HIPC(c, hipFree(c->d_w0frag[ln]));
              c->d_w0frag[ln] = nullptr; c->w0frag_cap[ln] = 0;
              HIPC(c, hipMalloc((void**)&c->d_w0frag[ln], need * sizeof(uint4)));
              c->w0frag_cap[ln] = need;
            }
            launch_w0gate(a.gate, a.w0t, a.c0, gate_rows, a.wparts, c->d_w0frag[ln], c->oor_cur + oi, v.stream());
            a.w0frag = c->d_w0frag[ln];
          }
        }
        if (deep) launch_mbxd(a, rows, o.k, o.stride, v.stream());
        else launch_mbxb(a, rows, o.k, o.stride, v.stream());
      } else {
        launch_mbx(a, rows, o.k, o.stride, v.stream());
      }
      break;
    }
    case UDA_OP_SEP: {
      const uda_buf_desc_t& ib = c->bufs[o.in[0]];
      if (c->wsplit_off[oi] < 0) return fail(c, "op %d: fused separable conv needs a split scheme (pw_scheme != f32)", oi);
      SepArgs a{};
      a.in = v.ptr(o.in[0]);
      a.out = v.ptr(o.out);
      a.wd = has_wpar(c, oi) ? (const float*)wpar_of(c, oi) : v.wt(o.w2_off);
      a.wsplit = wsplit_of(c, oi);
      a.wparts = c->wscheme[oi];
      a.wunscale = c->wunscale[oi];
      a.oor = c->oor_cur + oi;
      if (uda_split_f16(a.wparts)) c->oor_armed = true;
      a.bias = v.wt(o.bias_off);
      a.bn_scale = v.wt(o.bn_scale_off);
      a.bn_shift = v.wt(o.bn_shift_off);
      a.mask = v.mask(o.drop_site);
      a.mask_in = (!o.fuse_in && o.drop_site2 >= 0) ? v.mask(o.drop_site2) : nullptr;
      a.H = ob.H; a.W = ob.W; a.C = ib.C; a.Cout = ob.C;
      a.in_div = v.div(ib, ob);
      a.act = o.act;
      if (a.mask_in && !sep_tin_supported(a.C, a.Cout, a.wparts))
        return fail(c, "op %d: separable conv %d -> %d has no deferred-input mode (planner: plan.sep_tin_supported)", oi, a.C, a.Cout);
      if (o.fuse_in) {
        FuseArgs f{};
        if (int rc = fill_fuse_args(c, v, oi, f)) return rc;
        f.act = o.fuse_act;
        if (!sepf_supported(a.C, a.Cout, a.wparts)) return fail(c, "op %d: fused-input separable conv %d -> %d not supported", oi, a.C, a.Cout);
        a.in = nullptr;
        launch_sepf(a, f, rows, v.stream());
        break;
      }
      if (ib.H != ob.H || ib.W != ob.W) return fail(c, "op %d: separable conv changes the map size", oi);
      launch_sep(a, rows, v.stream());
      break;
    }
    case UDA_OP_SE: {
      const uda_buf_desc_t& pb = c->bufs[o.in[0]];
      const uda_buf_desc_t& src = c->bufs[o.in[1]];
      SeArgs a{};
      a.partial = v.ptr(o.in[0]);
      a.scale = v.ptr(o.out);
      a.w1 = v.wt(o.se_w1_off); a.b1 = v.wt(o.se_b1_off);
      a.w2 = v.wt(o.se_w2_off); a.b2 = v.wt(o.se_b2_off);
      a.C = src.C; a.mid = o.se_mid; a.n_tiles = pb.H * pb.W;
      a.inv_hw = 1.0f / (float)(src.H * src.W);
      if (pb.C != src.C || ob.C != src.C) return fail(c, "op %d: SE channel mismatch", oi);
      if (a.mid < 1 || a.mid > 1024) return fail(c, "op %d: SE hidden width %d outside [1, 1024]", oi, a.mid);
      a.mask = v.mask(o.drop_site);
      a.in_div = v.div(pb, ob);
      a.act = o.act;
      if (o.drop_site >= 0 && !ob.per_sample && c->model.mc_samples > 1) return fail(c, "op %d: deferred dropout needs a per-sample gate", oi);
      if (pb.per_sample != src.per_sample) return fail(c, "op %d: SE sums and source disagree on the sample axis", oi);
      launch_se(a, rows, v.stream());
      break;
    }
    case UDA_OP_FUSE:
    case UDA_OP_POOL: {
      FuseArgs a{};
      if (int rc = fill_fuse_args(c, v, oi, a)) return rc;
      if (a.C != ob.C) return fail(c, "op %d: fuse inputs have %d channels, output %d", oi, a.C, ob.C);
      a.out = v.ptr(o.out);
      a.act = o.act;
      a.total = (int64_t)rows * ob.H * ob.W * (ob.C / 4);
      launch_fuse(a, v.stream());
      break;
    }
    default:
      return fail(c, "op %d: unknown kind %d", oi, o.kind);
  }
  return 0;
}

static int run_sep_group(uda_ctx* c, const ChunkView& v, int oi, int n) {
  if (n < 2 || n > UDA_SEP_MAX_LV || oi + n > (int)c->ops.size()) return -1;
  const uda_op_t& o0 = c->ops[oi];
  const uda_buf_desc_t& ib0 = c->bufs[o0.in[0]];
  const uda_buf_desc_t& ob0 = c->bufs[o0.out];
  SepLevel lv[UDA_SEP_MAX_LV];
  for (int j = 0; j < n; ++j) {
    const uda_op_t& o = c->ops[oi + j];
    if (o.kind != UDA_OP_SEP || c->wsplit_off[oi + j] < 0) return -1;
    const uda_buf_desc_t& ib = c->bufs[o.in[0]];
    const uda_buf_desc_t& ob = c->bufs[o.out];
    if (ib.C != ib0.C || ob.C != ob0.C || o.act != o0.act || ib.per_sample != ib0.per_sample || ob.per_sample != ob0.per_sample ||
        ib.H != ob.H || ib.W != ob.W)
      return -1;
    for (int k = 0; k < n; ++k)
      if (k != j && (c->ops[oi + k].out == o.in[0] || c->ops[oi + k].out == o.out)) return -1;
    lv[j].in = v.ptr(o.in[0]);
    lv[j].out = v.ptr(o.out);
    lv[j].wd = has_wpar(c, oi + j) ? (const float*)wpar_of(c, oi + j) : v.wt(o.w2_off);
    lv[j].wsplit = wsplit_of(c, oi + j);
    lv[j].bias = v.wt(o.bias_off);
    lv[j].bn_scale = v.wt(o.bn_scale_off);
    lv[j].bn_shift = v.wt(o.bn_shift_off);
    lv[j].mask = v.mask(o.drop_site);
    lv[j].mask_in = o.drop_site2 >= 0 ? v.mask(o.drop_site2) : nullptr;
    if ((o.drop_site2 >= 0) != (o0.drop_site2 >= 0)) return -1;
    lv[j].H = ob.H; lv[j].W = ob.W;
    lv[j].wunscale = c->wunscale[oi + j];
    if (c->wscheme[oi + j] != c->wscheme[oi]) return -1;
  }
  for (int j = 0; j < n; ++j) {
    const uda_buf_desc_t& obj = c->bufs[c->ops[oi + j].out];
    const char* o0p = (const char*)lv[j].out;
    const char* o1p = o0p + (size_t)v.rows(obj) * obj.H * obj.W * obj.C * sizeof(float);
    for (int k = 0; k < n; ++k) {
      if (k == j) continue;
      const uda_buf_desc_t& ibk = c->bufs[c->ops[oi + k].in[0]];
      const uda_buf_desc_t& obk = c->bufs[c->ops[oi + k].out];
      const char* i0p = (const char*)lv[k].in;
      const char* i1p = i0p + (size_t)v.rows(ibk) * ibk.H * ibk.W * ibk.C * sizeof(float);
      const char* q0p = (const char*)lv[k].out;
      const char* q1p = q0p + (size_t)v.rows(obk) * obk.H * obk.W * obk.C * sizeof(float);
      if ((o0p < i1p && i0p < o1p) || (o0p < q1p && q0p < o1p))
        return fail(c, "ops %d and %d of a launch group overlap in memory (arena plan broken)", oi + j, oi + k);
    }
  }
  ProfScope ps(c, UDA_OP_SEP, v.stream(), n);
  SepArgs a{};
  a.C = ib0.C; a.Cout = ob0.C;
  a.in_div = v.div(ib0, ob0);
  a.act = o0.act;
  a.mask_in = o0.drop_site2 >= 0 ? v.mask(o0.drop_site2) : nullptr;
  if (a.mask_in && !sep_tin_supported(a.C, a.Cout, c->wscheme[oi]))
    return fail(c, "ops %d..: separable conv %d -> %d has no deferred-input mode (planner: plan.sep_tin_supported)", oi, a.C, a.Cout);
  a.wparts = c->wscheme[oi];
  a.wunscale = c->wunscale[oi];
  a.oor = c->oor_cur + oi;
  if (uda_split_f16(a.wparts)) c->oor_armed = true;
  launch_sep_multi(a, lv, n, v.rows(ob0), v.stream());
  return 0;
}

static int run_post_range(uda_ctx* c, int i0, int n, int post_mode, hipStream_t st);

static int run_preprocess(uda_ctx* c) {
  const uda_model_t& m = c->model;
  ProfScope ps(c, 18);
  PreprocArgs a{};
  const uda_ctx::U8Slot& sl = c->u8[c->cur];
  a.in = sl.d_img; a.out = c->d_images; a.geo = sl.d_geo;
  a.n = c->n_images; a.H = m.image_h; a.W = m.image_w;
  for (int k = 0; k < 3; ++k) { a.mean[k] = m.mean_rgb[k]; a.stdv[k] = m.stddev_rgb[k]; }
  if (c->noise_from >= 0) {
    PreprocArgs b = a;
    a.n = c->noise_from;
    b.n = c->n_images - c->noise_from;
    b.out = c->d_images + (size_t)c->noise_from * m.image_h * m.image_w * 3;
    b.noise = 1; b.noise_seed = c->seed; b.noise_img0 = (uint32_t)c->image_offset;
    launch_preprocess(a, c->stream);
    launch_preprocess(b, c->stream);
  } else {
    launch_preprocess(a, c->stream);
  }
  HIPC(c, hipGetLastError());
  c->pre_valid = true;
  return 0;
}

static int run_network(uda_ctx* c, int post_mode = 0, bool chunk_post = false, hipEvent_t defer_ev = nullptr) {
  const uda_model_t& m = c->model;
  const int n = c->n_images, T = m.mc_samples;
  bool stem_u8 = false;
  if (c->have_u8) {
    static const bool on = (uda_env_int("UDA_STEM_U8", 1) != 0);
    const uda_ctx::U8Slot& sl = c->u8[c->cur];
    stem_u8 = on && c->noise_from < 0 && c->stem_co > 0 && stem_u8_supported(c->stem_co) && c->stem_act == UDA_ACT_SWISH;
    for (int i = 0; i < n && stem_u8; ++i) stem_u8 = sl.geo[i].sh == sl.geo[i].h && sl.geo[i].sw == sl.geo[i].w;
    c->pre_valid = false;
    if (!stem_u8) {
      if (int rc = run_preprocess(c)) return rc;
      HIPC(c, hipEventRecord(c->ev_pre_done[c->cur], c->stream));
    }
  }
  c->stem_from_u8 = stem_u8;
  if (!c->sites.empty()) {
    const int rows = n * T;
    if (c->masks_injected && c->masks_rows != rows)
      return fail(c, "injected dropout masks cover %d sample rows, the run has %d", c->masks_rows, rows);
    int64_t off = 0;
    for (size_t s = 0; s < c->sites.size(); ++s) {
      c->site_off[s] = off;
      off += (int64_t)rows * c->sites[s].channels;
    }
    if (!c->masks_injected) {
      HIPC(c, hipMemcpyAsync(c->d_site_off, c->site_off.data(), c->sites.size() * sizeof(int64_t),
                             hipMemcpyHostToDevice, c->stream));
      launch_philox_masks(c->d_masks, c->d_site_off, c->d_site_ch, c->d_site_rate, (int)c->sites.size(), rows,
                          (uint32_t)(c->image_offset * (c->t_total > 0 ? c->t_total : T)), c->max_c4, c->seed,
                          T, c->t_total > 0 ? c->t_total : T, c->t_first, c->t_stride, c->stream);
    }
  }
  const int lanes = c->n_lanes;
  if (lanes > 1) {
    HIPC(c, hipEventRecord(c->ev_start, c->stream));
    for (int l = 1; l < lanes; ++l) HIPC(c, hipStreamWaitEvent(c->lane_stream[l], c->ev_start, 0));
  }
  int ci = 0;
  for (int i0 = 0; i0 < n; i0 += m.chunk_images, ++ci) {
    ChunkView v{c, i0, (n - i0 < m.chunk_images) ? n - i0 : m.chunk_images};
    v.lane = ci % lanes;
    bool gated = false;
    for (int oi = 0; oi < (int)c->ops.size(); ++oi) {
      if (c->gate_ev && !gated && c->bufs[c->ops[oi].out].kind >= 2) {
        HIPC(c, hipStreamWaitEvent(v.stream(), c->gate_ev, 0));
        gated = true;
      }
      const int grp = c->ops[oi].launch_group;
      if (grp > 1) {
        const int rg = run_sep_group(c, v, oi, grp);
        if (rg > 0) return rg;
        if (rg == 0) {
          const hipError_t le = hipGetLastError();
          if (le != hipSuccess)
            return fail(c, "ops %d..%d (head layer, one launch for %d pyramid levels): launch failed: %s", oi, oi + grp - 1, grp, hipGetErrorString(le));
          oi += grp - 1;
          continue;
        }
      }
      const int rc = run_op(c, v, oi);
      if (rc) return rc;
      static const bool sync_each = getenv("UDA_SYNC_EACH") != nullptr;
      if (sync_each) {
        const uda_op_t& o = c->ops[oi];
        fprintf(stderr, "[uda] op %d kind %d k %d s %d C %d -> %d ... ", oi, o.kind, o.k, o.stride, c->bufs[o.in[0]].C, c->bufs[o.out].C);
        fflush(stderr);
        const hipError_t se = hipStreamSynchronize(v.stream());
        fprintf(stderr, "%s\n", hipGetErrorString(se));
      }
      const hipError_t le = hipGetLastError();
      if (le != hipSuccess) {
        const uda_op_t& o = c->ops[oi];
        return fail(c, "op %d (kind %d, k %d, stride %d, in C %d, out C %d): launch failed: %s", oi, o.kind, o.k, o.stride,
                    c->bufs[o.in[0]].C, c->bufs[o.out].C, hipGetErrorString(le));
      }
    }
    c->last_chunk_i0 = i0;
    c->last_chunk_n = v.nc;
    c->last_lane = v.lane;
    if (chunk_post) {
      HIPC(c, hipEventRecord(c->ev_chunk[ci], v.stream()));
      HIPC(c, hipStreamWaitEvent(c->post_stream, c->ev_chunk[ci], 0));
      const int rc = run_post_range(c, i0, v.nc, post_mode, c->post_stream);
      if (rc) return rc;
    }
  }
  if (chunk_post) {
    if (defer_ev) {
      HIPC(c, hipEventRecord(defer_ev, c->post_stream));
    } else {
      HIPC(c, hipEventRecord(c->ev_post, c->post_stream));
      HIPC(c, hipStreamWaitEvent(c->stream, c->ev_post, 0));
    }
    c->last_post_mode = post_mode;
    c->last_n = n;
  }
  for (int l = 1; l < lanes; ++l) {
    HIPC(c, hipEventRecord(c->ev_done[l], c->lane_stream[l]));
    HIPC(c, hipStreamWaitEvent(c->stream, c->ev_done[l], 0));
  }
  if (stem_u8) HIPC(c, hipEventRecord(c->ev_pre_done[c->cur], c->stream));
  HIPC(c, hipGetLastError());
  return 0;
}

static NmsArgs nms_args_at(uda_ctx::NmsWs& w, size_t p0, int problems, int K, int M, const float* boxes);

bool run_nms(const NmsArgs& na, const float* scores, int M, hipStream_t st, uda_ctx::PrefixWs* pw, size_t p0, NmsCoop coop) {
  const int solo = solo_limit();
  static const int reg = uda_env_int("UDA_NMS_REG", 1);
  if (na.K <= solo && reg && nms_reg_supported(na)) {
    launch_nms_reg(na, scores, st);
    return false;
  }
  if (na.K <= solo && nms_solo_supported(na)) {
    launch_nms_solo(na, scores, st);
    return false;
  }
  static const int coop_on = uda_env_int("UDA_NMS_COOP", 1);
  if (coop_on && coop.bar && coop.err) {
    const int lc = launch_nms_coop(na, scores, coop.bar + p0 * nms_coop_slot_words(M), coop.err, st);
    if (lc > 0) {
      if (coop.used) *coop.used = true;
      return false;
    }
    if (lc < 0 && coop.not_launched) ++*coop.not_launched;
  }
  if (pw && pw->Lcap > 0 && na.segs == 1 && na.K > pw->Lcap && M <= 128) {
    const size_t lc = (size_t)pw->Lcap;
// ... 1088 lines not shown
```

### uncertainty-detection-autolabeling_amd/csrc/uda_ctx.h

```cpp
#pragma once
#include <stdint.h>

#include <string>
#include <utility>
#include <vector>

#include "uda_internal.h"

using namespace uda;

struct ProfSlot {
  double total_ms = 0;
  int64_t launches = 0;
  struct Pending { hipEvent_t first, second; int weight; };
  std::vector<Pending> pending;
};

struct uda_ctx {
  uda_model_t model;
  std::vector<uda_buf_desc_t> bufs;
  std::vector<uda_op_t> ops;
  std::vector<uda_drop_site_t> sites;
  int device = 0;
  hipStream_t stream = nullptr;
  std::string err;

  float* d_weights = nullptr;
  int64_t n_weights = 0;
  uint16_t* d_wsplit = nullptr;
  std::vector<int64_t> wsplit_off;
  std::vector<int64_t> wpar_off;
  int pw_parts = UDA_SPLIT_F16X2;
  std::vector<int> wscheme;
  std::vector<float> wunscale;
  std::vector<float> wascale;
  int n_f16_ops = 0, n_f16_demoted = 0;
  std::vector<char> buf_f16;
  unsigned* d_oor = nullptr;
  unsigned* oor_cur = nullptr;
  int oor_half = 0;
  bool oor_armed = false;
  std::vector<float> h_weights;
  std::vector<uint16_t*> wovr;
  std::vector<int64_t> wovr_par;
  int64_t range_demotions = 0;
  struct RunRec {
    bool valid = false, do_post = false, have_u8 = false, masks_injected = false;
    int pm = 0, cur = 0, n = 0;
    uint64_t slot_gen = 0, f32_gen = 0, masks_gen = 0, seed = 0;
    int64_t image_offset = 0;
  };
  RunRec last_run;
  const RunRec* replay_rec = nullptr;
  uint64_t f32_gen = 0, masks_gen = 0;
  float* d_arena = nullptr;
  uint4* d_w0frag[2] = {nullptr, nullptr};
  size_t w0frag_cap[2] = {0, 0};
  int n_lanes = 1;
  hipStream_t lane_stream[2] = {nullptr, nullptr};
  float* lane_arena[2] = {nullptr, nullptr};
  hipEvent_t ev_start = nullptr, ev_done[2] = {nullptr, nullptr};
  int last_lane = 0;
  hipStream_t post_stream = nullptr;
  std::vector<hipEvent_t> ev_chunk;
  hipEvent_t ev_post = nullptr;
  int post_overlap = 1;
  float* d_anchors = nullptr;
  int A_tot = 0;
  int a_off[UDA_MAX_LEVELS + 1];

  struct U8Slot {
    uint8_t* d = nullptr;
    size_t cap = 0;
    uint8_t* pinned = nullptr;
    size_t pcap = 0;
    int n = 0;
    bool valid = false, uploaded = false;
    uint64_t gen = 0;
    std::vector<PreGeo> geo;
    PreGeo* d_geo = nullptr;
    uint8_t* d_img = nullptr;
    std::vector<float> scales;
    hipEvent_t ev = nullptr;
  } u8[2];
  int cur = 0;
  hipStream_t copy_stream = nullptr;
  hipEvent_t ev_pre_done[2] = {nullptr, nullptr};
  bool have_u8 = false;
  int stem_act = UDA_ACT_SWISH;
  bool stem_from_u8 = false;
  bool pre_valid = false;
  int stem_co = 0;
  float* d_images = nullptr;
  float* d_scales = nullptr;
  int noise_from = -1;
  std::vector<PreGeo> cons_geo;
  double* d_cons_iou = nullptr;
  uint8_t* d_cons_agree = nullptr;
  int cons_n = 0;
  std::vector<float> h_scales;
  int n_images = 0;
  int sh = 0, sw = 0;

  float* d_masks = nullptr;
  int64_t mask_cap = 0;
  int64_t sum_site_ch = 0;
  int max_c4 = 0;
  std::vector<int64_t> site_off;
  int64_t* d_site_off = nullptr;
  int32_t* d_site_ch = nullptr;
  float* d_site_rate = nullptr;
  bool masks_injected = false;
  int masks_rows = 0;
// ... 37 lines not shown
  int64_t coop_not_launched = 0;
  unsigned long long* d_merge_keys = nullptr;
  float *d_oboxes = nullptr, *d_oscores = nullptr, *d_oclasses = nullptr, *d_ologits = nullptr;
  float *d_oprobs = nullptr, *d_oentropy = nullptr;
  float* d_opacked = nullptr;
  int32_t* d_ovalid = nullptr;
  float *d_gt_boxes = nullptr, *d_gt_classes = nullptr, *h_gt = nullptr;
  hipEvent_t gt_ev = nullptr;
  char* d_asg_pack = nullptr;
  std::vector<char> h_asg;
  float* d_asg_rows = nullptr;
  int gt_cap = 0, gt_n = 0, gt_G = 0;
  int asg_n = 0, asg_G = 0;
  int64_t asg_rows = -1;
  char* d_score_pack = nullptr;
  std::vector<char> h_score;
  int score_n = 0, score_nc = 0;
  bool score_fetched = false;
  char* d_pseudo_pack = nullptr;
  char* d_pseudo_slots = nullptr;
  std::vector<char> h_pseudo;
  int pseudo_n = 0, pseudo_cap = 0;
  bool pseudo_fetched = false;
  char* d_lc_pack = nullptr;
  std::vector<char> h_lc;
  int lc_cap = 0, lc_n = 0, lc_G = 0;
  bool lc_fetched = false;
  float *d_egt = nullptr, *h_egt = nullptr;
  hipEvent_t egt_ev = nullptr;
  char* d_eval_pack = nullptr;
  std::vector<char> h_eval;
  int egt_cap = 0, egt_n = 0, egt_G = 0;
  int eval_n = 0;
  bool eval_fetched = false;
  int last_post_mode = 0;
  int last_n = 0;
  int last_chunk_i0 = 0, last_chunk_n = 0;
  struct AsyncSlot {
    hipEvent_t ev = nullptr;
    bool open = false;
    bool joined = true;
    int64_t seq = 0;
    int n = 0, mode = 0;
    bool coop_used = false, oor_armed = false;
    bool cands_lost = false;
    RunRec rec;
    std::vector<std::pair<int, int>> pending;
    float *oboxes = nullptr, *oscores = nullptr, *oclasses = nullptr, *ologits = nullptr, *scales = nullptr;
    int32_t* ovalid = nullptr;
  };
  AsyncSlot as[2];
  int as_next = 0;
  int64_t as_seq = 0;
  bool as_ready = false;
  const float* d_scales_post = nullptr;
  hipStream_t aux_stream = nullptr;
  hipEvent_t gate_ev = nullptr;

  uint32_t prof_mask = 0;
  ProfSlot prof[32];
};

int fail(uda_ctx* c, const char* fmt, ...);

#define HIPC(ctx, expr)                                                                   \
  do {                                                                                    \
    hipError_t e_ = (expr);                                                               \
    if (e_ != hipSuccess)                                                                 \
      return fail(ctx, "%s: %s failed: %s (%s:%d)", __func__, #expr, hipGetErrorString(e_), __FILE__, __LINE__); \
  } while (0)

template <typename T>
inline hipError_t dalloc(T** p, size_t n) {
  return hipMalloc((void**)p, (n ? n : 1) * sizeof(T));
}

struct ProfScope {
  uda_ctx* c;
  int kind;
  hipStream_t st;
  hipEvent_t e0 = nullptr, e1 = nullptr;
  bool on;
  int weight;
  ProfScope(uda_ctx* c_, int kind_, hipStream_t st_ = nullptr, int weight_ = 1)
      : c(c_), kind(kind_), st(st_ ? st_ : c_->stream), weight(weight_) {
    on = (c->prof_mask >> kind) & 1u;
    if (on) {
      hipEventCreate(&e0);
      hipEventCreate(&e1);
      hipEventRecord(e0, st);
    }
  }
  ~ProfScope() {
    if (on) {
      hipEventRecord(e1, st);
      c->prof[kind].pending.push_back({e0, e1, weight});
    }
  }
};

inline int box_cols_of(const uda_model_t& m, int post_mode) {
  if (post_mode == UDA_POST_PER_CLASS) return 4;
  int cols = 4;
  if (m.has_uncert && m.loss_attenuation) cols += 4;
  if (m.has_uncert && m.box_stacked) cols += 4;
  return cols;
}
inline int cls_cols_of(const uda_model_t& m, int post_mode) {
  if (post_mode == UDA_POST_PER_CLASS) return 1;
  return 1 + ((m.has_uncert && m.cls_stacked) ? (m.max_nms_inputs > 0 ? 1 : m.num_classes) : 0);
}

struct NmsCoop {
  unsigned long long* bar = nullptr;
  int* err = nullptr;
  bool* used = nullptr;
  int64_t* not_launched = nullptr;
};

int finish_post(uda_ctx* c);
int ensure_probs(uda_ctx* c, int rows);
bool run_nms(const NmsArgs& na, const float* scores, int M, hipStream_t st, uda_ctx::PrefixWs* pw = nullptr, size_t p0 = 0,
             NmsCoop coop = NmsCoop());
void nms_params(NmsArgs& a, float iou_thr, float score_thr, float soft_sigma);
int solo_limit();
int prefix_target();
hipError_t alloc_prefix_ws(uda_ctx::PrefixWs& w, size_t problems, int Lcap, size_t M);
void free_prefix_ws(uda_ctx::PrefixWs& w);
```

### uncertainty-detection-autolabeling_amd/csrc/uda_internal.h

```cpp
#pragma once
#include <hip/hip_runtime.h>
#include <stdint.h>
#include <stdlib.h>

#include "../../include/uda_hip.h"

namespace uda {

#ifdef __HIPCC__
__device__ __forceinline__ void philox4x32_10(uint32_t c0, uint32_t c1, uint32_t c2, uint32_t c3,
                                              uint32_t k0, uint32_t k1, uint32_t out[4]) {
#pragma unroll
  for (int r = 0; r < 10; ++r) {
    const uint64_t p0 = (uint64_t)0xD2511F53u * c0;
    const uint64_t p1 = (uint64_t)0xCD9E8D57u * c2;
    const uint32_t n0 = (uint32_t)(p1 >> 32) ^ c1 ^ k0;
    const uint32_t n1 = (uint32_t)p1;
    const uint32_t n2 = (uint32_t)(p0 >> 32) ^ c3 ^ k1;
    const uint32_t n3 = (uint32_t)p0;
    c0 = n0; c1 = n1; c2 = n2; c3 = n3;
    k0 += 0x9E3779B9u;
    k1 += 0xBB67AE85u;
  }
  out[0] = c0; out[1] = c1; out[2] = c2; out[3] = c3;
// ... 92 lines not shown
  const float* mask_in;
  int H, W, C, Cout;
  int in_div;
  int act;
  int wparts;
  float wunscale;
  unsigned* oor;
};
void launch_sep(const SepArgs& a, int rows, hipStream_t s);
bool sep_tin_supported(int C, int Cout, int scheme);
constexpr int UDA_SEP_MAX_LV = 8;
struct SepLevel {
  const float* in; float* out; const float* wd; const void* wsplit;
  const float* bias; const float* bn_scale; const float* bn_shift; const float* mask; const float* mask_in;
  int H, W;
  float wunscale;
};
struct SepMulti {
  SepArgs one;
  int n_lv;
  int tiles, rows;
  int tile0[UDA_SEP_MAX_LV + 1];
  SepLevel lv[UDA_SEP_MAX_LV];
};
void launch_sep_multi(const SepArgs& common, const SepLevel* lv, int n_lv, int rows, hipStream_t s);
bool sep_supported(int C, int Cout);
size_t sep_lds_bytes(int C, int Cout, int scheme, bool tin = false);
struct FuseArgs;
void launch_sepf(const SepArgs& a, const FuseArgs& fused, int rows, hipStream_t s);
bool sepf_supported(int C, int Cout, int scheme);
size_t sepf_lds_bytes(int C, int Cout, int scheme);

struct DwArgs {
  const float* in;
  float* out;
  const float* w;
  const float* bn_scale;
  const float* bn_shift;
  const float* mask;
  float* se_partial;
  int H, W, Ho, Wo, C;
  int pad_t, pad_l;
  int in_div;
  int act;
  int tc;
  int pxb;
  int n_cchunk;
  int n_tiles;
};

struct MbxArgs {
  const float* in;
  float* out;
  int out_f16;
  const float* we;
  const float* sc0;
  const float* sh0;
  const float* mask0;
  const float* wd;
  const float* sc1;
  const float* sh1;
  const float* mask1;
  float* se_partial;
  int H, W, Ho, Wo, Cin, Cmid;
  int pad_t, pad_l;
  int in_div;
  int n_tiles;
  const void* wsplit;
  int wparts;
  unsigned* oor;
  const float* wpar;
  const float* gate;
  const float* w0t;
  const float* sh0f;
  const uint4* w0frag;
  int c0, g_div;
  int remap_T, tiles_x, tiles_y;
  int ch_groups;
};
void mbxb_pack_proj(const float* w0, const float* sc, const float* sh, int c0, int cout, float* out);
size_t mbx_par_floats(int Cmid, int k);
void mbx_pack_params(const float* wd, const float* sc1, const float* sh1, int Cmid, int k, float* out);
void launch_mbxb(const MbxArgs& a, int rows, int k, int stride, hipStream_t s);
void launch_mbxd(const MbxArgs& a, int rows, int k, int stride, hipStream_t s);
bool mbxd_supported(int Cin, int Cmid, int k, int stride);
size_t mbx_lds_bytes(int Cin, int Cmid, int k, int stride, int scheme, int Ho, int Wo);
int mbxd_tiles(int Ho, int Wo, int k, int stride = 1);
bool mbxd_wide(int Ho, int Wo, int k, int stride);
bool mbxb_supported(int Cin, int Cmid, int k, int stride);
int mbxb_tiles(int Ho, int Wo, int k, int stride);
size_t mbxb_packed_elems(int Cin, int Cmid, int scheme = UDA_SPLIT_BF16X2);
size_t mbxb_w0frag_elems(int gate_rows, int scheme);
void launch_w0gate(const float* gate, const float* w0t, int c0, int gate_rows, int scheme, uint4* out, unsigned* oor, hipStream_t s);
void mbxb_pack_weights(const float* we, const float* sc0, const float* sh0, int Cin, int Cmid, uint16_t* out, bool perm16 = false,
                       int scheme = UDA_SPLIT_BF16X2, float* stats = nullptr);
void launch_mbx(const MbxArgs& a, int rows, int k, int stride, hipStream_t s);
int mbx_tiles(int Ho, int Wo, int k, int stride);
bool mbx_supported(int Cin, int Cmid, int k, int stride);

struct SeArgs {
  const float* partial;
  float* scale;
  const float* w1;
  const float* b1;
  const float* w2;
  const float* b2;
  int C, mid, n_tiles;
  float inv_hw;
  const float* mask;
  int in_div;
  int act;
};

struct FuseArgs {
  const float* in[UDA_MAX_FUSE_INPUTS];
  float* out;
  float wgt[UDA_MAX_FUSE_INPUTS];
  int mode[UDA_MAX_FUSE_INPUTS];
  int Hi[UDA_MAX_FUSE_INPUTS], Wi[UDA_MAX_FUSE_INPUTS];
  int in_div[UDA_MAX_FUSE_INPUTS];
  float sy[UDA_MAX_FUSE_INPUTS], sx[UDA_MAX_FUSE_INPUTS];
  int pk[UDA_MAX_FUSE_INPUTS], ps[UDA_MAX_FUSE_INPUTS];
  int ppt[UDA_MAX_FUSE_INPUTS], ppl[UDA_MAX_FUSE_INPUTS];
  int n_in;
  int H, W, C;
  int act;
  int64_t total;
};

void launch_stem(const StemArgs& a, hipStream_t s);
bool stem_u8_supported(int Co);
void launch_pw(const PwArgs& a, int rows, hipStream_t s);
void launch_dw(DwArgs a, int rows, int k, int stride, hipStream_t s);
void dw_geometry(int C, int Wo, int k, int stride, int* tc, int* pxb, int* n_cchunk, int* grid_x, int* xb);
int dw_tiles(int C, int Ho, int Wo, int k, int stride);
void launch_se(const SeArgs& a, int rows, hipStream_t s);
void launch_fuse(const FuseArgs& a, hipStream_t s);
void launch_philox_masks(float* masks, const int64_t* site_off_dev, const int32_t* site_ch_dev,
                         const float* site_rate_dev, int n_sites, int rows, uint32_t row_base, int max_c4,
                         uint64_t seed, int t_local, int t_total, int t_first, int t_stride, hipStream_t s);

struct LevelTable {
  int num_levels;
  int hw[UDA_MAX_LEVELS];
  int a_off[UDA_MAX_LEVELS + 1];
  const float* cls[UDA_MAX_LEVELS];
  const float* box[UDA_MAX_LEVELS];
};

struct AggArgs {
  LevelTable lv;
  const float* anchors;
  int n_img, A_tot, A, C;
  int K;
  const int32_t* cand_flat;
  int Tc, Tb;
  int loss_att;
  int decode;
  float* boxes;
  float* scores;
  int32_t* classes;
  float* logits;
  float* u_cls;
  float* u_al;
  float* u_ep;
  int park_all, cls_slots;
// ... 373 lines not shown
```

### uncertainty-detection-autolabeling_amd/plan.py

```python
import os

import numpy as np

from . import arch, capi
from .hparams_config import get_feat_sizes, parse_image_size

ALIGN = 256


def dw_tiles_x(C, Wo, k, stride):
    C4 = C // 4
    cap = 16 if k == 5 else 64
    ncc = (C4 + cap - 1) // cap
    t = (C4 + ncc - 1) // ncc
    p = max(1, 256 // t)
    x = 1 if k == 5 else (4 if stride == 1 else 2)
    need = (Wo + x - 1) // x
    p = min(p, need)
    if k == 5:
        nb = (need + p - 1) // p
        p = (need + nb - 1) // nb
    return (Wo + p * x - 1) // (p * x)


def dw_rows(k, stride):
    return 16 if (k == 5 and stride == 1) else 8


def dw_tiles(C, Ho, Wo, k, stride):
    return -(-Ho // dw_rows(k, stride)) * dw_tiles_x(C, Wo, k, stride)


PW_SCHEMES = ("f16x2", "bf16x3", "bf16x2", "f32", "f16")
PW_SCHEME_DEFAULT = "f16x2"
PW_SCHEME_CODES = {"f32": 0, "bf16x2": 2, "bf16x3": 3, "f16x2": 4, "f16": 5}

PLAN_SWITCHES = {"UDA_DEFER_DROPOUT": 1, "UDA_FUSE_SEP": 1, "UDA_FUSE_PROJ": 1, "UDA_FUSE_MBX": 1, "UDA_FUSE_MBX6": 1,
                 "UDA_FUSE_MBXD": 1, "UDA_FUSE_IN": 1, "UDA_SEP_MULTI": 1}


def pw_scheme():
    v = os.environ.get("UDA_PW_SCHEME")
    if v:
        if v not in PW_SCHEMES:
            raise ValueError("UDA_PW_SCHEME=%r: expected one of %s" % (v, ", ".join(PW_SCHEMES)))
        return v
    t = os.environ.get("UDA_PW_TERMS")
    if t is None or t == "":
        return PW_SCHEME_DEFAULT
    t = int(t)
    if t not in (0, 3, 6):
        raise ValueError("UDA_PW_TERMS=%r: expected 6, 3 or 0" % (t,))
    return {0: "f32", 3: "bf16x2", 6: "bf16x3"}[t]


def split_pieces(sch):
    return {"bf16x3": 3, "f16": 1}.get(sch, 2)


def mbx_deep(cin):
    return cin > 48


def mbx_tile(k, stride, cin, Ho, Wo, sch):
    if mbx_deep(cin):
        if stride == 1:
            normal, wide = ((12, 16), (8, 20)) if k == 3 else ((8, 16), (6, 20))
            slots = lambda t: -(-Ho // t[0]) * t[0] * -(-Wo // t[1]) * t[1]
            return wide if slots(wide) < slots(normal) else normal
        return (7, 8) if k == 3 else (4, 10)
    if sch == "f32":
        return (8, 16) if stride == 1 else ((4, 16) if k == 3 else (4, 8))
    return ((12, 16) if k == 3 else (8, 16)) if stride == 1 else ((7, 8) if k == 3 else (4, 10))


def mbx_tiles(Ho, Wo, k, stride, cin, sch):
    th, tw = mbx_tile(k, stride, cin, Ho, Wo, sch)
    return -(-Ho // th) * -(-Wo // tw)


def mbx_supported(cin, cmid, k, stride, sch):
    if not (cin % 8 == 0 and cmid % 4 == 0 and k in (3, 5) and stride in (1, 2)):
        return False
    if mbx_deep(cin):
        return sch != "f32" and (cin + 1 + 15) // 16 in (6, 8, 13, 14)
    return 16 <= cin


def sepf_supported(C, Cout, sch):
    if sch == "f32":
        return False
    npc = split_pieces(sch)
    lds = 18 * 18 * 36 * 4 + 2 * (-(-Cout // 32)) * npc * 1024
    return C % 8 == 0 and 16 <= C <= 128 and Cout % 4 == 0 and 4 <= Cout <= 128 and lds <= 80 * 1024


def sep_tin_supported(C, Cout, sch):
    if sch == "f32":
        return False
    if C % 8 or not 64 <= C <= 128 or Cout < 1:
        return False
    ks, ntl, npc = -(-C // 16), -(-Cout // 32), split_pieces(sch)
    if not 2 <= ntl <= 4:
        return False
    a_img = 128 * (ks * 64 + 16) if sch == "bf16x3" else npc * 128 * (ks * 32 + 16)
    stg = 4 * 32 * ntl * 32 * 4 if Cout % 4 else 4 * 32 * 68 * 4
    if sch == "f16":
        a_img = max(a_img, stg)
    return stg <= a_img and a_img + ks * ntl * npc * 1024 <= 120 * 1024


def same_out(n, s):
    return -(-n // s)


ACT_CODES = {"swish": capi.ACT_SWISH, "silu": capi.ACT_SWISH, "swish_native": capi.ACT_SWISH,
             "relu": capi.ACT_RELU, "relu6": capi.ACT_RELU6, "hswish": capi.ACT_HSWISH, "mish": capi.ACT_MISH}
MODEL_PARAM_HANDLING = {
    "name": "inert: a label (the structure comes from the keys below)",
    "backbone_name": "consumed: arch.backbone_blocks (efficientnet-b0..b7; anything else raises)",
    "backbone_config": "consumed: arch.backbone_blocks (custom block table)",
    "image_size": "consumed", "num_classes": "consumed", "min_level": "consumed", "max_level": "consumed",
    "num_scales": "consumed", "aspect_ratios": "consumed", "anchor_scale": "consumed",
    "mean_rgb": "consumed", "stddev_rgb": "consumed",
    "box_class_repeats": "consumed", "fpn_cell_repeats": "consumed", "fpn_num_filters": "consumed",
    "act_type": "consumed: swish | silu | swish_native | relu | relu6 | hswish | mish; srelu raises (utils.py:42-59)",
    "separable_conv": "checked: False (dense 3x3 convs in BiFPN and heads) raises",
    "apply_bn_for_resampling": "consumed (efficientdet_keras.py:313-318)",
    "conv_after_downsample": "consumed (efficientdet_keras.py:331-338)",
    "conv_bn_act_pattern": "consumed (efficientdet_keras.py:218,229-236)",
    "fpn_name": "checked: None | bifpn | bifpn_dyn; qufpn raises",
    "fpn_weight_method": "consumed: fastattn | attn | sum; channel_attn / channel_fastattn raise",
    "fpn_config": "checked: None, or {nodes, weight_method} with at most three inputs per node",
    "heads": "checked: must be ['object_detection'] (segmentation head is not on the path)",
    "data_format": "checked: channels_last only",
    "survival_prob": "inert: drop_connect acts under training=True only (efficientdet_keras.py:464-465)",
    "is_training_bn": "inert: BN layers run with training=False at inference (moving statistics)",
    "strategy": "inert: selects the BN class / TPU placement, same inference arithmetic",
    "mixed_precision": "inert: the HIP path always computes in float32-class arithmetic (a superset)",
    "grad_checkpoint": "inert: training memory option",
    "loss_attenuation": "consumed", "uncert_adjust_method": "consumed (l-norm | n-flow | falsedec | sample; else raises)",
    "decode_nsamples": "consumed", "mc_dropout": "consumed", "mc_dropoutrate": "consumed", "mc_classheadrate": "consumed",
    "mc_boxheadrate": "consumed", "mc_dropoutsamp": "consumed", "enable_softmax": "consumed",
    "nms_configs": "consumed (method hard | gaussian; anything else raises; pyfunc is served by uda_nms_np)",
    "tflite_max_detections": "inert: TFLite export only",
    "max_instances_per_image": "inert: training / eval padding",
    "clip_min_uncert": "inert: loss only", "clip_max_uncert": "inert: loss only",
    "calibrate_classification": "consumed by calibration.py (above the driver)", "calib_method_class": "consumed by calibration.py",
    "calibrate_regression": "consumed by calibration.py", "calib_method_box": "consumed by calibration.py",
    "infer_draw_uncert": "consumed by visualize", "label_map": "consumed by infer_lib / writers",
    "consistency_ssl": "consumed: infer_lib plans 4 x batch_size images for serve_consistency (flip / blur / noise "
                       "variants, infer_model.py:768-848); writers.predict_to_file writes cons_iou / cons_cls",
    "assign_gt_box": "consumed: default method of ServingDriver.assign_ground_truth / serve_validate (IoU | MSE | else the GT "
                     "row's own rank; utils_extra.py:44-64, validate_model.py:337, calibrate_model.py:140)",
    "thr_fpr_tpr": "consumed by thresholding (budget of the ROC search)",
    "thr_cd": "consumed by thresholding (budget on correct / missing detections, else on false ones)",
    "thr_iou_thrs": "consumed by thresholding (IoU thresholds the weights are optimised over)",
    "thr_sel_uncert": "consumed by thresholding.from_validate_records (ENT and / or ALBOX)",
    "early_stopping_patience": "inert: training",
    "count_classes": "inert: training", "boxloss_type": "inert: training", "save_freq": "inert: training",
    "sample_images": "inert: training", "sample_images_freq": "inert: training", "save_train_images": "inert: training",
    "autoaugment_policy": "inert: training", "map_freq": "inert: training", "box_loss_weight": "inert: training",
    "moving_average_decay": "consumed by weights.resolve_weights (EMA shadows)",
}


def act_code(cfg):
    name = cfg.get("act_type", "swish")
    if name in ACT_CODES:
# ... 7 lines not shown
    lo, hi = cfg["min_level"], cfg["max_level"]
    fc = cfg.get("fpn_config")
    if fc:
        fc = fc if isinstance(fc, dict) else fc.as_dict()
        nodes = [dict(feat_level=int(n["feat_level"]), inputs_offsets=[int(o) for o in n["inputs_offsets"]]) for n in fc["nodes"]]
        for n in fc["nodes"]:
            if n.get("weight_method") not in (None, fc.get("weight_method")):
                raise ValueError("fpn_config: per-node weight_method (qufpn) is not available on the HIP path")
        return nodes, fc.get("weight_method") or "fastattn"
    name = cfg.get("fpn_name")
    if name not in (None, "", "bifpn", "bifpn_dyn"):
        if name == "qufpn":
            raise ValueError("fpn_name 'qufpn' is not available on the HIP path (bifpn only)")
        raise KeyError(name)
    return arch.bifpn_nodes(lo, hi), cfg.get("fpn_weight_method") or "fastattn"


def check_model_params(cfg):
    act_code(cfg)
    if not cfg.get("separable_conv", True):
        raise ValueError("separable_conv=False (dense 3x3 convolutions in the BiFPN and the heads) is not available on the HIP path")
    if cfg.get("data_format", "channels_last") != "channels_last":
        raise ValueError("data_format %r: the HIP path is NHWC (channels_last) only" % (cfg.get("data_format"),))
    heads = cfg.get("heads") or ["object_detection"]
    if list(heads) != ["object_detection"]:
        raise ValueError("heads %r: only ['object_detection'] is on the HIP path" % (list(heads),))
    nodes, method = fpn_nodes(cfg)
    if method not in ("fastattn", "attn", "sum"):
        if method in ("channel_attn", "channel_fastattn"):
            raise ValueError("fpn weight_method %r (per-channel fusion weights) is not available on the HIP path" % method)
        raise ValueError("unknown weight_method %s" % method)
    lo, hi = cfg["min_level"], cfg["max_level"]
    for n in nodes:
        if not 1 <= len(n["inputs_offsets"]) <= capi.MAX_FUSE:
            raise ValueError("fpn node with %d inputs: the HIP fusion takes 1..%d" % (len(n["inputs_offsets"]), capi.MAX_FUSE))
        if not lo <= n["feat_level"] <= hi:
            raise ValueError("fpn node at level %d outside [%d, %d]" % (n["feat_level"], lo, hi))
    unknown = sorted(k for k in cfg if k not in MODEL_PARAM_HANDLING and not k.startswith("uda_"))
    return unknown


class _Buf:
    __slots__ = ("H", "W", "C", "per_sample", "kind", "level", "offset", "first", "last", "name", "storage")

    def __init__(self, H, W, C, per_sample, kind=0, level=0, name=""):
        self.H, self.W, self.C, self.per_sample = int(H), int(W), int(C), bool(per_sample)
        self.kind, self.level, self.offset = kind, level, 0
        self.first, self.last, self.name = None, None, name
        self.storage = "f32"


class Plan:

    def __init__(self, config, weights, chunk_images=1, max_images=1, post_only=False):
        self.cfg = dict(config)
        self.unknown_keys = check_model_params(self.cfg)
        self.act = act_code(self.cfg)
        self.post_only = bool(post_only)
        self.w = weights
        self.T = arch.mc_flags(self.cfg)[2]
        self.cls_stacked, self.box_stacked, _ = arch.mc_flags(self.cfg)
        self.sample_axis = self.T > 1 or bool(self.cfg.get("uda_force_sample_axis"))
        self.chunk_images = int(chunk_images)
        self.max_images = int(max_images)
        self.bufs, self.ops, self.blob, self.blob_len = [], [], [], 0
        self.sites = []
        self.site_index = {}
        self.buffer_names = {}
        self.pw_scheme = self.cfg.get("uda_pw_scheme") or pw_scheme()
        if self.pw_scheme not in PW_SCHEMES:
            raise ValueError("uda_pw_scheme=%r: expected one of %s" % (self.pw_scheme, ", ".join(PW_SCHEMES)))
        sw = self.sw = {k: int(os.environ.get(k, d)) for k, d in PLAN_SWITCHES.items()}
        split = self.pw_scheme != "f32"
        self.defer_dropout = bool(sw["UDA_DEFER_DROPOUT"])
        self.fuse_sep = bool(sw["UDA_FUSE_SEP"]) and split
        self.fuse_proj = bool(sw["UDA_FUSE_PROJ"]) and split and bool(sw["UDA_FUSE_MBX"])
        self.fuse_in = self.fuse_sep and bool(sw["UDA_FUSE_IN"])
        self.defer_head = self.fuse_sep
        if self.post_only:
            self._post_only_layout()
            return
        self._build_sites()
        self._lower()
        self._plan_memory()
        self.mark_f16_storage()

    def _post_only_layout(self):
        cfg = self.cfg
        fs = get_feat_sizes(cfg["image_size"], cfg["max_level"])
        self.level_hw = [tuple(fs[l]) for l in range(cfg["min_level"], cfg["max_level"] + 1)]
        self.cls_stacked_dev = bool(self.cls_stacked and self.sample_axis)
        self.box_stacked_dev = bool(self.box_stacked and self.sample_axis)
        self._buf(1, 1, 4, False, name="unused")
        self.arena_floats = ALIGN
        self.fpn_out, self.head_out = [], {"class": [], "box": []}

    def _pack(self, arr):
        arr = np.ascontiguousarray(arr, dtype=np.float32).reshape(-1)
        off = self.blob_len
        pad = (-arr.size) % 4
        self.blob.append(arr)
        if pad:
            self.blob.append(np.zeros(pad, np.float32))
        self.blob_len += arr.size + pad
        return off

    def _bn(self, prefix):
        g, b = self.w[prefix + "/gamma"], self.w[prefix + "/beta"]
        m, v = self.w[prefix + "/moving_mean"], self.w[prefix + "/moving_variance"]
        scale = (g / np.sqrt(v + np.float32(arch.BN_EPS))).astype(np.float32)
        shift = (b - m * scale).astype(np.float32)
        return self._pack(scale), self._pack(shift)

    def _build_sites(self):
        cfg = self.cfg
        if not cfg["mc_dropout"]:
            return
        r_bb, r_cls, r_box = arch.dropout_rates(cfg)
        for i, b in enumerate(arch.backbone_blocks(cfg["backbone_name"], cfg.get("backbone_config"))):
            mid = b["cin"] * b["expand"]
            if b["expand"] != 1:
                self.sites.append(("blocks_%d/expand" % i, mid, r_bb))
            self.sites.append(("blocks_%d/dw" % i, mid, r_bb))
        F = cfg["fpn_num_filters"]
        for tag, r in (("class", r_cls), ("box", r_box)):
            for i in range(cfg["box_class_repeats"]):
                for lvl in range(cfg["min_level"], cfg["max_level"] + 1):
                    self.sites.append(("%s-%d-%d" % (tag, i, lvl), F, r))
        self.site_index = {name: i for i, (name, _, _) in enumerate(self.sites)}

    def _site(self, name):
        if name not in self.site_index:
            return -1
        i = self.site_index[name]
        return i if self.sites[i][2] > 0 else -1

    def _buf(self, H, W, C, per_sample, kind=0, level=0, name=""):
        self.bufs.append(_Buf(H, W, C, per_sample and self.sample_axis, kind, level, name))
        if name:
            self.buffer_names[name] = len(self.bufs) - 1
        return len(self.bufs) - 1

    def _op(self, kind, ins, out, **kw):
        o = dict(kind=kind, ins=list(ins), out=out, se_scale=-1, se_partial=-1, residual=-1, k=0,
                 stride=1, act=capi.ACT_NONE, w_off=-1, bias_off=-1, bn_scale_off=-1, bn_shift_off=-1,
                 se_w1_off=-1, se_b1_off=-1, se_w2_off=-1, se_b2_off=-1, se_mid=0, drop_site=-1,
                 resample=[0, 0, 0], fuse_w=[0.0, 0.0, 0.0], drop_site2=-1, w2_off=-1, bn2_scale_off=-1,
                 bn2_shift_off=-1, launch_group=0, fuse_in=0, fuse_act=capi.ACT_NONE)
        o.update(kw)
        self.ops.append(o)
        return out

    def _pw(self, x, cout, kernel, name, bias=None, bn=None, act=capi.ACT_NONE, site=-1, se=-1,
            residual=-1, out_kind=0, level=0):
        xb = self.bufs[x]
        ps = xb.per_sample or site >= 0 or (se >= 0 and self.bufs[se].per_sample)
        out = self._buf(xb.H, xb.W, cout, ps, out_kind, level, name)
        kw = dict(w_off=self._pack(self.w[kernel]), act=act, drop_site=site, se_scale=se, residual=residual)
        if bias is not None:
            kw["bias_off"] = self._pack(self.w[bias])
        if bn is not None:
            kw["bn_scale_off"], kw["bn_shift_off"] = self._bn(bn)
        return self._op(capi.OP_PW, [x], out, **kw)

    def _dw(self, x, k, stride, kernel, name, bn=None, act=capi.ACT_NONE, site=-1, with_se=False, defer_site=False):
        xb = self.bufs[x]
# ... 194 lines not shown
                for i, off in enumerate(node["inputs_offsets"]):
                    xi, mode = self._resample(cell[off], tgt.H, tgt.W, p + "resample_%d_%d_%d" % (i, off, nf),
                                              "cell%d/fnode%d/in%d" % (rep, n, i))
                    ins.append(xi)
                    modes.append(mode)
                if method == "fastattn":
                    ew = [np.maximum(np.float32(np.asarray(w[p + "WSM" + ("" if i == 0 else "_%d" % i)]).reshape(())), np.float32(0))
                          for i in range(len(ins))]
                    tot = np.float32(0)
                    for e in ew:
                        tot = np.float32(tot + e)
                    fw = [float(np.float32(e / np.float32(tot + np.float32(0.0001)))) for e in ew]
                elif method == "attn":
                    ev = np.asarray([np.asarray(w[p + "WSM" + ("" if i == 0 else "_%d" % i)], np.float32).reshape(())
                                     for i in range(len(ins))], np.float32)
                    ex = np.exp(ev - ev.max(), dtype=np.float32)
                    fw = [float(v) for v in (ex / ex.sum(dtype=np.float32)).astype(np.float32)]
                elif method == "sum":
                    fw = [1.0] * len(ins)
                else:
                    raise ValueError("unknown weight_method %s" % method)
                ps = any(self.bufs[i].per_sample for i in ins)
                op = p + "op_after_combine%d" % nf
                fuse_act, conv_act = (capi.ACT_NONE, self.act) if cba else (self.act, capi.ACT_NONE)
                bias = None if cba else op + "/conv/bias"
                if self.fuse_in and sepf_supported(F, F, self.pw_scheme):
                    cell.append(self._sepconv(None, F, op + "/conv/depthwise_kernel", op + "/conv/pointwise_kernel",
                                              "cell%d/fnode%d/out" % (rep, n), bias=bias, bn=op + "/bn", act=conv_act,
                                              fusion=dict(ins=ins, resample=modes, fuse_w=fw, H=tgt.H, W=tgt.W, act=fuse_act)))
                    continue
                fused = self._op(capi.OP_FUSE, ins, self._buf(tgt.H, tgt.W, F, ps, name="cell%d/fnode%d/fused" % (rep, n)),
                                 act=fuse_act, resample=(modes + [0, 0, 0])[:3], fuse_w=(fw + [0, 0, 0])[:3])
                cell.append(self._sepconv(fused, F, op + "/conv/depthwise_kernel", op + "/conv/pointwise_kernel",
                                          "cell%d/fnode%d/out" % (rep, n), bias=bias, bn=op + "/bn", act=conv_act))
            feats = []
            for lvl in range(lo, hi + 1):
                for i, node in enumerate(reversed(nodes)):
                    if node["feat_level"] == lvl:
                        feats.append(cell[-1 - i])
                        break
        self.fpn_out = list(feats)
        self.level_hw = [(self.bufs[f].H, self.bufs[f].W) for f in feats]
        A = len(cfg["aspect_ratios"]) * cfg["num_scales"]
        cls_ch = A * cfg["num_classes"]
        box_ch = A * (8 if cfg["loss_attenuation"] else 4)
        self.head_out = {"class": [], "box": []}
        for net, tag, outc, kind in (("class_net", "class", cls_ch, 2), ("box_net", "box", box_ch, 3)):
            xs = list(feats)
            pending = [-1] * len(feats)
            nrep = cfg["box_class_repeats"]
            for i in range(nrep):
                pre = "%s/%s-%d" % (net, tag, i)
                first = len(self.ops)
                next_cout = F if i + 1 < nrep else outc
                for li in range(len(feats)):
                    site = self._site("%s-%d-%d" % (tag, i, lo + li))
                    defer = (site >= 0 and pending[li] < 0 and not self.bufs[xs[li]].per_sample
                             and self.defer_head and sep_tin_supported(F, next_cout, self.pw_scheme))
                    xs[li] = self._sepconv(xs[li], F, pre + "/depthwise_kernel", pre + "/pointwise_kernel",
                                           "%s-%d-%d" % (tag, i, lo + li), bias=pre + "/bias",
                                           bn="%s/%s-%d-bn-%d" % (net, tag, i, lo + li), act=self.act,
                                           site=-1 if defer else site, in_site=pending[li])
                    pending[li] = site if defer else -1
                self._mark_launch_group(first)
            pre = "%s/%s-predict" % (net, tag)
            first = len(self.ops)
            for li in range(len(feats)):
                out = self._sepconv(xs[li], outc, pre + "/depthwise_kernel", pre + "/pointwise_kernel",
                                    "%s-predict-%d" % (tag, lo + li), bias=pre + "/bias", out_kind=kind, level=li,
                                    in_site=pending[li])
                self.head_out[tag].append(out)
            self._mark_launch_group(first)
        for tag, stacked in (("class", self.cls_stacked), ("box", self.box_stacked)):
            for o in self.head_out[tag]:
                want = bool(stacked and self.sample_axis)
                if self.bufs[o].per_sample != want:
                    assert not self.bufs[o].per_sample, "unexpected sample axis on head %s" % tag
        self.cls_stacked_dev = bool(self.bufs[self.head_out["class"][0]].per_sample)
        self.box_stacked_dev = bool(self.bufs[self.head_out["box"][0]].per_sample)

    def _rows(self, b):
        return self.chunk_images * (self.T if b.per_sample else 1)

    def _plan_memory(self):
        for oi, o in enumerate(self.ops):
            touched = list(o["ins"]) + [o["out"]] + [o[k] for k in ("se_scale", "se_partial", "residual") if o[k] >= 0]
            for b in touched:
                buf = self.bufs[b]
                if buf.first is None:
                    buf.first = oi
                buf.last = oi
        for f in self.fpn_out:
            self.bufs[f].last = len(self.ops)
        if self.cfg.get("uda_keep_buffers"):
            for b in self.bufs:
                if b.first is not None:
                    b.last = len(self.ops)
        for oi, o in enumerate(self.ops):
            n = o.get("launch_group", 0)
            if n > 1:
                end = oi + n - 1
                for g in self.ops[oi:oi + n]:
                    for b in list(g["ins"]) + [g["out"]]:
                        buf = self.bufs[b]
                        buf.last = max(buf.last, end)
                        buf.first = min(buf.first, oi)
        free, top = [], 0

        def alloc(size):
            nonlocal top
            for i, (off, sz) in enumerate(free):
                if sz >= size:
                    if sz == size:
                        free.pop(i)
                    else:
                        free[i] = (off + size, sz - size)
                    return off
            off = top
            top += size
            return off

        def release(off, size):
            free.append((off, size))
            free.sort()
            merged = []
            for o_, s_ in free:
                if merged and merged[-1][0] + merged[-1][1] == o_:
                    merged[-1] = (merged[-1][0], merged[-1][1] + s_)
                else:
                    merged.append((o_, s_))
            free[:] = merged

        sizes = {}
        for oi in range(len(self.ops)):
            for bi, b in enumerate(self.bufs):
                if b.kind == 0 and b.first == oi:
                    size = -(-(self._rows(b) * b.H * b.W * b.C) // ALIGN) * ALIGN
                    sizes[bi] = size
                    b.offset = alloc(size)
            for bi, b in enumerate(self.bufs):
                if b.kind == 0 and b.last == oi and bi in sizes:
                    release(b.offset, sizes[bi])
        self.arena_floats = int(top)

    def anchors(self):
        cfg = self.cfg
        lo, hi = cfg["min_level"], cfg["max_level"]
        H, W = parse_image_size(cfg["image_size"])
        fs = get_feat_sizes(cfg["image_size"], hi)
        scales = cfg["anchor_scale"]
        if not isinstance(scales, (list, tuple)):
            scales = [scales] * (hi - lo + 1)
        levels = []
        for lvl in range(lo, hi + 1):
            sy, sx = H / float(fs[lvl][0]), W / float(fs[lvl][1])
            ys = np.arange(sy / 2, H, sy)
            xs = np.arange(sx / 2, W, sx)
            yv, xv = np.meshgrid(ys, xs, indexing="ij")
            per = []
            for octave in range(cfg["num_scales"]):
                for aspect in cfg["aspect_ratios"]:
                    base_x = scales[lvl - lo] * sx * 2 ** (octave / float(cfg["num_scales"]))
                    base_y = scales[lvl - lo] * sy * 2 ** (octave / float(cfg["num_scales"]))
                    if isinstance(aspect, (list, tuple)):
                        ax, ay = aspect
                    else:
                        ax = np.sqrt(aspect)
                        ay = 1.0 / ax
                    hx, hy = base_x * ax / 2.0, base_y * ay / 2.0
                    per.append(np.stack([yv - hy, xv - hx, yv + hy, xv + hx], axis=-1))
            levels.append(np.stack(per, axis=2).reshape(-1, 4))
        return np.concatenate(levels).astype(np.float32)

    def to_c(self, post_mode=capi.POST_GLOBAL):
        cfg = self.cfg
        H, W = parse_image_size(cfg["image_size"])
        m = capi.Model()
        m.abi_version = capi.UDA_ABI_VERSION
        m.image_h, m.image_w = H, W
        mean, std = cfg["mean_rgb"], cfg["stddev_rgb"]
        if not isinstance(mean, (list, tuple)):
            mean, std = [mean] * 3, [std] * 3
        for i in range(3):
            m.mean_rgb[i] = np.float32(mean[i])
            m.stddev_rgb[i] = np.float32(std[i])
        m.num_levels = len(self.level_hw)
        for i, (h, w_) in enumerate(self.level_hw):
            m.level_h[i], m.level_w[i] = h, w_
        m.anchors_per_loc = len(cfg["aspect_ratios"]) * cfg["num_scales"]
        m.num_classes = cfg["num_classes"]
        m.loss_attenuation = int(bool(cfg["loss_attenuation"]))
        m.mc_samples = self.T
        m.cls_stacked = int(self.cls_stacked_dev)
        m.box_stacked = int(self.box_stacked_dev)
        m.has_uncert = int(bool(cfg["loss_attenuation"] or cfg["mc_dropout"]))
        method = cfg["uncert_adjust_method"]
        if not cfg["loss_attenuation"]:
            m.decode_method = capi.DECODE_PLAIN
        elif method in ("l-norm", "n-flow"):
            m.decode_method = capi.DECODE_LNORM
        elif method == "falsedec":
            m.decode_method = capi.DECODE_FALSEDEC
        elif method == "sample":
            m.decode_method = capi.DECODE_SAMPLE
            m.decode_nsamples = int(cfg.get("decode_nsamples", 100))
            if not 1 <= m.decode_nsamples <= 4096:
                raise ValueError("decode_nsamples must be in [1, 4096]")
        else:
            raise ValueError("uncert_adjust_method %r is not available on the HIP path" % method)
        m.enable_softmax = int(bool(cfg["enable_softmax"]))
        sigma2, iou, thr = nms_params(cfg)
        m.nms_soft_sigma, m.nms_iou_thresh, m.nms_score_thresh = sigma2, iou, thr
        m.max_output_size = int(cfg["nms_configs"]["max_output_size"])
        m.max_nms_inputs = int(cfg["nms_configs"].get("max_nms_inputs", 0) or 0)
        m.post_mode = post_mode
        m.chunk_images, m.max_images = self.chunk_images, self.max_images
        m.arena_floats = self.arena_floats
        m.n_drop_sites = len(self.sites)
        m.pw_scheme = PW_SCHEME_CODES[self.pw_scheme]

        bufs = (capi.BufDesc * len(self.bufs))()
        for i, b in enumerate(self.bufs):
            bufs[i].H, bufs[i].W, bufs[i].C = b.H, b.W, b.C
            bufs[i].per_sample = int(b.per_sample)
            bufs[i].offset, bufs[i].kind, bufs[i].level = int(b.offset), b.kind, b.level
        ops = (capi.Op * max(1, len(self.ops)))()
        for i, o in enumerate(self.ops):
            c = ops[i]
            c.kind = o["kind"]
            ins = (o["ins"] + [-1, -1, -1])[:3]
            for j in range(3):
                c.in_[j] = ins[j]
                c.resample[j] = o["resample"][j]
                c.fuse_w[j] = o["fuse_w"][j]
            c.n_in = len(o["ins"])
            for k in ("out", "se_scale", "se_partial", "residual", "k", "stride", "act", "w_off", "bias_off",
                      "bn_scale_off", "bn_shift_off", "se_w1_off", "se_b1_off", "se_w2_off", "se_b2_off",
                      "se_mid", "drop_site", "drop_site2", "w2_off", "bn2_scale_off", "bn2_shift_off", "launch_group"):
                setattr(c, k, int(o[k]))
            c.fuse_in = int(o.get("fuse_in", 0))
            c.fuse_act = int(o.get("fuse_act", 0))
        sites = (capi.DropSite * max(1, len(self.sites)))()
        for i, (_, ch, r) in enumerate(self.sites):
            sites[i].channels, sites[i].rate = ch, np.float32(r)
        blob = np.concatenate(self.blob) if self.blob else np.zeros(4, np.float32)
        return m, bufs, ops, sites, blob, self.anchors()

    def mark_f16_storage(self):
        for b in self.bufs:
            b.storage = "f32"
        if self.pw_scheme != "f16":
            return
        refs, ok = [0] * len(self.bufs), [0] * len(self.bufs)
        for o in self.ops:
            for j, b in enumerate(o["ins"]):
                if b >= 0:
                    refs[b] += 1
                    ok[b] += int((j == 0 and o["kind"] == capi.OP_PW) or (j == 1 and o["kind"] == capi.OP_SE))
            for key in ("se_scale", "se_partial", "residual"):
                if o[key] >= 0:
                    refs[o[key]] += 1
        for o in self.ops:
            b = o["out"]
            if o["kind"] == capi.OP_MBX and self.bufs[b].kind == 0 and refs[b] > 0 and refs[b] == ok[b]:
                self.bufs[b].storage = "f16"

    def summary(self):
        return dict(n_ops=len(self.ops), n_bufs=len(self.bufs), arena_mb=self.arena_floats * 4 / 2 ** 20,
                    weights_mb=self.blob_len * 4 / 2 ** 20, sites=len(self.sites), T=self.T)


def nms_params(cfg):
    nc = cfg["nms_configs"]
    method = nc["method"]
    if method == "hard" or not method:
        return 0.0, float(nc["iou_thresh"] or 0.5), float(nc["score_thresh"] or float("-inf"))
    if method == "gaussian":
        return float(nc["sigma"] or 0.5) / 2, 0.5, float(nc["score_thresh"] or 0.001)
    raise ValueError("Inference has invalid nms method {}".format(method))


def op_costs(plan, n_images):
    import math
    T = plan.T
    chunks = math.ceil(n_images / plan.chunk_images)
    out = {}

    def size(bi):
        b = plan.bufs[bi]
        return n_images * (T if b.per_sample else 1) * b.H * b.W * b.C

    for o in plan.ops:
        ob = plan.bufs[o["out"]]
        rows = n_images * (T if ob.per_sample else 1)
        by = size(o["out"])
        fl = 0
        for bi in (o["ins"][:1] if o["kind"] == capi.OP_SE else o["ins"]):
            by += size(bi)
        for key in ("se_scale", "residual", "se_partial"):
            if o[key] >= 0 and o["kind"] != capi.OP_SE:
                by += size(o[key])
        k = o["kind"]
        if k == capi.OP_PW:
            cin = plan.bufs[o["ins"][0]].C
            by += cin * ob.C
            fl = 2 * rows * ob.H * ob.W * cin * ob.C
        elif k == capi.OP_DW:
            by += o["k"] * o["k"] * ob.C
            fl = 2 * rows * ob.H * ob.W * ob.C * o["k"] * o["k"]
        elif k == capi.OP_STEM:
            by += 27 * ob.C
            fl = 2 * rows * ob.H * ob.W * 27 * ob.C
        elif k == capi.OP_MBX:
            ib = plan.bufs[o["ins"][0]]
            cin = o["se_mid"] if o["se_scale"] >= 0 else ib.C
            by += cin * ob.C + o["k"] * o["k"] * ob.C
            fl = 2 * rows * (ib.H * ib.W * cin * ob.C + ob.H * ob.W * ob.C * o["k"] * o["k"])
            if o["se_scale"] >= 0:
                by += ib.C * cin
                fl += 2 * rows * ib.H * ib.W * ib.C * cin
        elif k == capi.OP_SEP:
            ib = plan.bufs[o["ins"][0]]
            by += ib.C * ob.C + 9 * ib.C
            fl = 2 * rows * ob.H * ob.W * (9 * ib.C + ib.C * ob.C)
            if o.get("fuse_in"):
# ... 11 lines not shown
```

Baseline: 5240.

## Split chunk into half-batches and co-launch MBX with narrow PW in one kernel

Adds a half-batch window schedule for runs of PW→(MBX, SE)* blocks. The chunk is split into two halves that are offset by one stage, so the projection PW of one half can be paired with the depthwise MBX of the other half. The pair is issued as a single heterogeneous kernel whose blocks dispatch to either the PW or the MBX body. The aim is to fill the GPU with small, low-occupancy narrow-PW launches and cut launch count. In exchange it adds a plan-table gate, an ABI field, longer buffer lifetimes and larger shared-LDS sizing for the paired kernel.

```diff
diff --git a/include/uda_hip.h b/include/uda_hip.h
--- a/include/uda_hip.h
+++ b/include/uda_hip.h
@@ -57,6 +57,7 @@
   int32_t launch_group;
   int32_t fuse_in;
   int32_t fuse_act;
+  int32_t half_win;
 } uda_op_t;
 
 typedef struct uda_drop_site {
diff --git a/uncertainty-detection-autolabeling_amd/capi.py b/uncertainty-detection-autolabeling_amd/capi.py
--- a/uncertainty-detection-autolabeling_amd/capi.py
+++ b/uncertainty-detection-autolabeling_amd/capi.py
@@ -52,7 +52,8 @@
                 ("drop_site", C.c_int32), ("resample", C.c_int32 * MAX_FUSE),
                 ("fuse_w", C.c_float * MAX_FUSE), ("n_in", C.c_int32), ("drop_site2", C.c_int32),
                 ("w2_off", C.c_int64), ("bn2_scale_off", C.c_int64), ("bn2_shift_off", C.c_int64),
-                ("launch_group", C.c_int32), ("fuse_in", C.c_int32), ("fuse_act", C.c_int32)]
+                ("launch_group", C.c_int32), ("fuse_in", C.c_int32), ("fuse_act", C.c_int32),
+                ("half_win", C.c_int32)]
 
 
 class DropSite(C.Structure):
diff --git a/uncertainty-detection-autolabeling_amd/csrc/kernels_pwb.hip b/uncertainty-detection-autolabeling_amd/csrc/kernels_pwb.hip
--- a/uncertainty-detection-autolabeling_amd/csrc/kernels_pwb.hip
+++ b/uncertainty-detection-autolabeling_amd/csrc/kernels_pwb.hip
@@ -9,24 +9,27 @@
 
 namespace uda {
 
-template <int MT, int NT, int WM, int WN, int PARTS, int OCC, bool DEEP = false>
-__global__ __launch_bounds__(256, OCC) void pwb_kernel(PwArgs a) {
+template <int MT, int NT, int WM, int WN, int PARTS>
+__host__ __device__ constexpr int pwb_lds_bytes() {
+  constexpr int ab = split_np(PARTS) * 32 * MT * WM * PWB_AROW + 2 * NT * WN * split_np(PARTS) * 1024;
+  constexpr int stg = 4 * 32 * PWB_STG * 4;
+  return ab > stg ? ab : stg;
+}
+
+template <int MT, int NT, int WM, int WN, int PARTS, bool DEEP>
+__device__ __forceinline__ void pwb_body(const PwArgs a, const dim3 bid, unsigned char* lds) {
   static_assert(WM * WN == 4, "four waves per block");
   constexpr int NPC = split_np(PARTS);
   constexpr int BM = 32 * MT * WM, NTB = NT * WN, BN = 32 * NTB;
   constexpr int A_BYTES = NPC * BM * PWB_AROW;
-  constexpr int B_BYTES = 2 * NTB * NPC * 1024;
-  constexpr int STG_BYTES = 4 * 32 * PWB_STG * 4;
-  constexpr int LDS_BYTES = (A_BYTES + B_BYTES) > STG_BYTES ? (A_BYTES + B_BYTES) : STG_BYTES;
-  __shared__ __attribute__((aligned(16))) unsigned char lds[LDS_BYTES];
   unsigned char* As = lds;
   uint4* Bs = (uint4*)(lds + A_BYTES);
 
   const int tid = threadIdx.x, lane = tid & 63, wave = tid >> 6;
   const int li = lane & 31, lh = lane >> 5;
   const int wr = wave / WN, wc = wave % WN;
-  const int bx = blockIdx.x, by = blockIdx.y;
-  const int b = blockIdx.z, b_in = b / a.in_div;
+  const int bx = bid.x, by = bid.y;
+  const int b = bid.z, b_in = b / a.in_div;
   const int m0 = bx * BM, n0 = by * BN;
   const int nt0 = by * NTB;
   const float* A = a.in + (size_t)b_in * a.HW * a.Cin;
@@ -264,6 +267,12 @@
       __syncthreads();
     }
   }
+}
+
+template <int MT, int NT, int WM, int WN, int PARTS, int OCC, bool DEEP = false>
+__global__ __launch_bounds__(256, OCC) void pwb_kernel(PwArgs a) {
+  __shared__ __attribute__((aligned(16))) unsigned char lds[pwb_lds_bytes<MT, NT, WM, WN, PARTS>()];
+  pwb_body<MT, NT, WM, WN, PARTS, DEEP>(a, dim3(blockIdx.x, blockIdx.y, blockIdx.z), lds);
 }
 
 __global__ __launch_bounds__(256, 3) void pwb_shared_kernel(PwArgs a) {
@@ -600,8 +609,8 @@
 #define UDA_MBXB_MINW(K, S, KSF, PARTS) ((PARTS) == 3 ? (((KSF) <= 2 && (K) == 3) ? UDA_MBXB6_W : 2) : \
     ((KSF) <= 2 ? ((K) == 3 ? 4 : 3) : (((KSF) <= 3 && ((K) == 3 ? (S) == 2 : UDA_MBXB_WK_LDS)) ? 3 : 2)))
 #endif
-template <int K, int S, int KSF, bool FUSE0, int PARTS, bool OH = false>
-__global__ __launch_bounds__(256, UDA_MBXB_MINW(K, S, KSF, PARTS)) void mbxb_kernel(MbxArgs a) {
+template <int K, int S, int KSF, bool FUSE0, int PARTS, bool OH>
+__device__ __forceinline__ void mbxb_body(const MbxArgs a, const dim3 bid, float* mlds) {
   constexpr int NW = 4;
   constexpr int NPC = split_np(PARTS);
   constexpr int TH = mbxb_cfg(K, S).th, TW = mbxb_cfg(K, S).tw;
@@ -620,7 +629,6 @@
   constexpr int NUNIT = TH * UPR;
   static_assert(TW % XW == 0, "units must tile the output tile");
   constexpr int NCOL = (XW - 1) * S + K;
-  extern __shared__ __attribute__((aligned(16))) float mlds[];
   float* E = mlds;
   float* red = E + (ET ? (size_t)32 * CP : (size_t)NPP * ES);
   constexpr int NPAR = (K * K + 2) * 32;
@@ -631,10 +639,10 @@
 
   const int tid = threadIdx.x, lane = tid & 63, wave = tid >> 6;
   const int li = lane & 31, lh = lane >> 5;
-  int tbx = blockIdx.x, tby = blockIdx.y, b = blockIdx.z;
+  int tbx = bid.x, tby = bid.y, b = bid.z;
   if (a.remap_T > 0) {
     const int T = a.remap_T, nt = a.tiles_x * a.tiles_y, ntp = (nt + 7) & ~7;
-    const unsigned L = blockIdx.x;
+    const unsigned L = bid.x;
     const unsigned per_img = (unsigned)ntp * (unsigned)T;
     const int img = (int)(L / per_img);
     const unsigned r = L - (unsigned)img * per_img;
@@ -928,6 +936,33 @@
 #pragma unroll
         for (int p_ = 0; p_ < NPC; ++p_) rb[ks][p_] = nbr[ks][p_];
     }
+  }
+}
+
+template <int K, int S, int KSF, bool FUSE0, int PARTS, bool OH = false>
+__global__ __launch_bounds__(256, UDA_MBXB_MINW(K, S, KSF, PARTS)) void mbxb_kernel(MbxArgs a) {
+  extern __shared__ __attribute__((aligned(16))) float mlds[];
+  mbxb_body<K, S, KSF, FUSE0, PARTS, OH>(a, dim3(blockIdx.x, blockIdx.y, blockIdx.z), mlds);
+}
+
+struct PairGrid {
+  unsigned mgx, mgy;
+  unsigned pgx, pgy;
+  unsigned n_pw, n;
+};
+template <int K, int S, int KSF, int PARTS, int NT>
+__global__ __launch_bounds__(256, UDA_MBXB_MINW(K, S, KSF, PARTS)) void mbx_pw_pair_kernel(MbxArgs ma, PwArgs pa, PairGrid pg) {
+  extern __shared__ __attribute__((aligned(16))) float pair_lds[];
+  const unsigned i = blockIdx.x;
+  const unsigned before = (unsigned)(((unsigned long long)i * pg.n_pw) / pg.n);
+  const unsigned after = (unsigned)(((unsigned long long)(i + 1) * pg.n_pw) / pg.n);
+  if (after != before) {
+    const unsigned x = before % pg.pgx, r = before / pg.pgx;
+    pwb_body<1, NT, 4, 1, PARTS, false>(pa, dim3(x, r % pg.pgy, r / pg.pgy), (unsigned char*)pair_lds);
+  } else {
+    const unsigned j = i - before;
+    const unsigned x = j % pg.mgx, r = j / pg.mgx;
+    mbxb_body<K, S, KSF, false, PARTS, false>(ma, dim3(x, r % pg.mgy, r / pg.mgy), pair_lds);
   }
 }
 
@@ -1024,6 +1059,48 @@
   else if (a.wparts == UDA_SPLIT_F16X2) launch_mbxb_p<4>(a, rows, k, stride, s);
   else if (a.wparts == UDA_SPLIT_F16X1) launch_mbxb_p<5>(a, rows, k, stride, s);
   else launch_mbxb_p<2>(a, rows, k, stride, s);
+}
+
+template <int K, int S, int KSF, int PARTS, int NT>
+static bool launch_pair_t(const MbxArgs& m, int mrows, const PwArgs& p, int prows, hipStream_t s) {
+  constexpr int TH = mbxb_cfg(K, S).th, TW = mbxb_cfg(K, S).tw;
+  constexpr int IH = (TH - 1) * S + K, IW = (TW - 1) * S + K;
+  constexpr int NPP = (IH * IW + 31) / 32 * 32;
+  constexpr size_t mlds = ((mbx_et_w(K, S) ? (size_t)32 * mbx_et_pitch(mbx_et_w(K, S)) : (size_t)NPP * 32) + 8 * 32 + 2 * (K * K + 2) * 32) * sizeof(float) +
+                          (size_t)KSF * split_np(PARTS) * 64 * sizeof(uint4);
+  constexpr size_t plds = (size_t)pwb_lds_bytes<1, NT, 4, 1, PARTS>();
+  PairGrid g;
+  g.mgx = (m.Wo + TW - 1) / TW; g.mgy = (m.Ho + TH - 1) / TH;
+  g.pgx = (p.HW + 127) / 128; g.pgy = (p.Cout + 32 * NT - 1) / (32 * NT);
+  const long long n_mbx = (long long)g.mgx * g.mgy * mrows, n_pw = (long long)g.pgx * g.pgy * prows;
+  if (n_mbx + n_pw >= (1ll << 31) || n_mbx <= 0 || n_pw <= 0) return false;
+  g.n_pw = (unsigned)n_pw; g.n = (unsigned)(n_mbx + n_pw);
+  MbxArgs b = m;
+  b.remap_T = 0;
+  hipLaunchKernelGGL((mbx_pw_pair_kernel<K, S, KSF, PARTS, NT>), dim3(g.n), dim3(256), mlds > plds ? mlds : plds, s, b, p, g);
+  return true;
+}
+template <int PARTS, int NT>
+static bool launch_pair_p(const MbxArgs& m, int mrows, int k, int stride, const PwArgs& p, int prows, hipStream_t s) {
+  const int ksf = (m.Cin + 1 + 15) / 16;
+  if (k == 3 && stride == 1 && ksf == 2) return launch_pair_t<3, 1, 2, PARTS, NT>(m, mrows, p, prows, s);
+  if (k == 5 && stride == 2 && ksf == 2) return launch_pair_t<5, 2, 2, PARTS, NT>(m, mrows, p, prows, s);
+  if (k == 5 && stride == 1 && ksf == 3) return launch_pair_t<5, 1, 3, PARTS, NT>(m, mrows, p, prows, s);
+  if (k == 3 && stride == 2 && ksf == 3) return launch_pair_t<3, 2, 3, PARTS, NT>(m, mrows, p, prows, s);
+  return false;
+}
+bool mbx_pw_pair_supported(const MbxArgs& m, int mrows, int k, int stride, const PwArgs& p) {
+  const int ksf = (m.Cin + 1 + 15) / 16;
+  if (m.gate || m.out_f16 || !m.wsplit || (m.wparts != UDA_SPLIT_F16X2 && m.wparts != UDA_SPLIT_BF16X3) || m.in_div != 1) return false;
+  if (!mbxb_supported(m.Cin, m.Cmid, k, stride)) return false;
+  if (!((k == 3 && stride == 1 && ksf == 2) || (k == 5 && stride == 2 && ksf == 2) || (k == 5 && stride == 1 && ksf == 3) || (k == 3 && stride == 2 && ksf == 3))) return false;
+  if (p.wparts != m.wparts || !p.wsplit || p.Cout > 64 || p.in_div != 1 || p.in_f16 || p.Cin >= 256) return false;
+  return true;
+}
+bool launch_mbx_pw_pair(const MbxArgs& m, int mrows, int k, int stride, const PwArgs& p, int prows, hipStream_t s) {
+  if (!mbx_pw_pair_supported(m, mrows, k, stride, p)) return false;
+  if (m.wparts == UDA_SPLIT_F16X2) return p.Cout <= 32 ? launch_pair_p<4, 1>(m, mrows, k, stride, p, prows, s) : launch_pair_p<4, 2>(m, mrows, k, stride, p, prows, s);
+  return p.Cout <= 32 ? launch_pair_p<3, 1>(m, mrows, k, stride, p, prows, s) : launch_pair_p<3, 2>(m, mrows, k, stride, p, prows, s);
 }
 
 struct MbxCfgD { int th, tw, xw; };
diff --git a/uncertainty-detection-autolabeling_amd/csrc/uda_api.hip b/uncertainty-detection-autolabeling_amd/csrc/uda_api.hip
--- a/uncertainty-detection-autolabeling_amd/csrc/uda_api.hip
+++ b/uncertainty-detection-autolabeling_amd/csrc/uda_api.hip
@@ -292,6 +292,20 @@
       uda_destroy(c);
       return 1;
     }
+  }
+  c->half_win_ok.assign(n_ops, 0);
+  for (int i = 0; i < n_ops; ++i) {
+    const int nw = ops[i].kind == UDA_OP_PW ? ops[i].half_win : 0;
+    if (nw <= 0) continue;
+    bool ok = nw % 3 == 0 && i + nw <= n_ops;
+    for (int q = 0; ok && q < nw; ++q) {
+      const uda_op_t& o = ops[i + q];
+      const int want = q % 3 == 0 ? UDA_OP_PW : (q % 3 == 1 ? UDA_OP_MBX : UDA_OP_SE);
+      ok = o.kind == want && bufs[o.out].kind == 0 && bufs[o.in[0]].kind == 0 && (q == 0 || o.kind != UDA_OP_PW || o.half_win == 0);
+    }
+    if (!ok) { fail(nullptr, "op %d: half-batch window of %d ops is not PW (MBX SE PW)* MBX SE on arena buffers", i, nw); uda_destroy(c); return 1; }
+    c->half_win_ok[i] = 1;
+    i += nw - 1;
   }
   for (int i = 0; i < n_bufs; ++i) {
     const uda_buf_desc_t& b = bufs[i];
@@ -748,6 +762,10 @@
   uda_ctx* c;
   int i0, nc;
   int lane = 0;
+  int sub0 = 0;
+  int prof_weight = 1;
+  PwArgs* cap_pw = nullptr;
+  MbxArgs* cap_mbx = nullptr;
   hipStream_t stream() const { return c->lane_stream[lane]; }
   int rows(const uda_buf_desc_t& b) const { return nc * (b.per_sample ? c->model.mc_samples : 1); }
   float* ptr(int id) const {
@@ -758,7 +776,7 @@
       case 1: return c->d_images + (size_t)i0 * per;
       case 2: return c->d_cls[b.level] + (size_t)i0 * (b.per_sample ? T : 1) * per;
       case 3: return c->d_box[b.level] + (size_t)i0 * (b.per_sample ? T : 1) * per;
-      default: return c->lane_arena[lane] + b.offset;
+      default: return c->lane_arena[lane] + b.offset + (size_t)sub0 * (b.per_sample ? T : 1) * per;
     }
   }
   const float* wt(int64_t off) const { return off < 0 ? nullptr : c->d_weights + off; }
@@ -819,7 +837,7 @@
   const uda_op_t& o = c->ops[oi];
   const uda_buf_desc_t& ob = c->bufs[o.out];
   const int rows = v.rows(ob);
-  ProfScope ps(c, o.kind, v.stream());
+  ProfScope ps(c, o.kind, v.stream(), v.prof_weight, !v.cap_pw && !v.cap_mbx);
   switch (o.kind) {
     case UDA_OP_STEM: {
       const uda_buf_desc_t& ib = c->bufs[o.in[0]];
@@ -876,8 +894,10 @@
         a.wunscale = c->wunscale[oi];
         a.oor = c->oor_cur + oi;
         if (uda_split_f16(a.wparts)) c->oor_armed = true;
+        if (v.cap_pw) { *v.cap_pw = a; return 0; }
         launch_pwb(a, rows, v.stream());
       } else {
+        if (v.cap_pw) return 0;
         launch_pw(a, rows, v.stream());
       }
       break;
@@ -946,6 +966,10 @@
         if (uda_split_f16(a.wparts)) c->oor_armed = true;
         a.wpar = (const float*)wpar_of(c, oi);
         a.out_f16 = c->buf_f16[o.out];
+        if (v.cap_mbx) {
+          if (!fuse0 && !deep) *v.cap_mbx = a;
+          return 0;
+        }
         if (fuse0) {
           const uda_buf_desc_t& gb = c->bufs[o.se_scale];
           if (gb.per_sample && !ob.per_sample) return fail(c, "op %d: per-sample gate on a per-image output", oi);
@@ -972,6 +996,7 @@
         if (deep) launch_mbxd(a, rows, o.k, o.stride, v.stream());
         else launch_mbxb(a, rows, o.k, o.stride, v.stream());
       } else {
+        if (v.cap_mbx) return 0;
         launch_mbx(a, rows, o.k, o.stride, v.stream());
       }
       break;
@@ -1136,6 +1161,49 @@
   return 0;
 }
 
+static int run_half_window(uda_ctx* c, const ChunkView& v, int ws, int n) {
+  const int nA = (v.nc + 1) / 2;
+  ChunkView h[2] = {v, v};
+  h[0].nc = nA;
+  h[1].i0 = v.i0 + nA; h[1].nc = v.nc - nA; h[1].sub0 = v.sub0 + nA;
+  h[1].prof_weight = 0;
+  auto both = [&](int hm, int om, int hp, int op, bool share) -> int {
+    if (share) {
+      PwArgs pa{};
+      MbxArgs ma{};
+      ChunkView vp = h[hp], vm = h[hm];
+      vp.cap_pw = &pa;
+      vm.cap_mbx = &ma;
+      if (int rc = run_op(c, vp, op)) return rc;
+      if (int rc = run_op(c, vm, om)) return rc;
+      if (pa.wsplit && ma.wsplit) {
+        const uda_op_t& mo = c->ops[om];
+        ProfScope ps(c, UDA_OP_MBX, v.stream(), h[hm].prof_weight);
+        if (launch_mbx_pw_pair(ma, h[hm].rows(c->bufs[mo.out]), mo.k, mo.stride, pa, h[hp].rows(c->bufs[c->ops[op].out]), v.stream())) return 0;
+      }
+    }
+    if (int rc = run_op(c, h[hp], op)) return rc;
+    return run_op(c, h[hm], om);
+  };
+  if (int rc = run_op(c, h[0], ws)) return rc;
+  const int blocks = n / 3;
+  for (int j = 0; j < blocks; ++j) {
+    const int om = ws + 1 + 3 * j, os = om + 1;
+    const int bits = c->ops[om].half_win;
+    if (int rc = both(0, om, 1, om - 1, (bits & 1) != 0)) return rc;
+    if (int rc = run_op(c, h[0], os)) return rc;
+    if (j + 1 < blocks) {
+      if (int rc = both(1, om, 0, om + 2, (bits & 2) != 0)) return rc;
+    } else {
+      if (int rc = run_op(c, h[1], om)) return rc;
+    }
+    if (int rc = run_op(c, h[1], os)) return rc;
+  }
+  const hipError_t le = hipGetLastError();
+  if (le != hipSuccess) return fail(c, "ops %d..%d (half-batch window): launch failed: %s", ws, ws + n - 1, hipGetErrorString(le));
+  return 0;
+}
+
 static int run_network(uda_ctx* c, int post_mode = 0, bool chunk_post = false, hipEvent_t defer_ev = nullptr) {
   const uda_model_t& m = c->model;
   const int n = c->n_images, T = m.mc_samples;
@@ -1183,6 +1251,12 @@
       if (c->gate_ev && !gated && c->bufs[c->ops[oi].out].kind >= 2) {
         HIPC(c, hipStreamWaitEvent(v.stream(), c->gate_ev, 0));
         gated = true;
+      }
+      if (c->half_win_ok[oi] && v.nc >= 2) {
+        const int nw = c->ops[oi].half_win;
+        if (int rc = run_half_window(c, v, oi, nw)) return rc;
+        oi += nw - 1;
+        continue;
       }
       const int grp = c->ops[oi].launch_group;
       if (grp > 1) {
diff --git a/uncertainty-detection-autolabeling_amd/csrc/uda_ctx.h b/uncertainty-detection-autolabeling_amd/csrc/uda_ctx.h
--- a/uncertainty-detection-autolabeling_amd/csrc/uda_ctx.h
+++ b/uncertainty-detection-autolabeling_amd/csrc/uda_ctx.h
@@ -29,6 +29,7 @@
   int64_t n_weights = 0;
   uint16_t* d_wsplit = nullptr;
   std::vector<int64_t> wsplit_off;
+  std::vector<char> half_win_ok;
   std::vector<int64_t> wpar_off;
   int pw_parts = UDA_SPLIT_F16X2;
   std::vector<int> wscheme;
@@ -232,9 +233,9 @@
   hipEvent_t e0 = nullptr, e1 = nullptr;
   bool on;
   int weight;
-  ProfScope(uda_ctx* c_, int kind_, hipStream_t st_ = nullptr, int weight_ = 1)
+  ProfScope(uda_ctx* c_, int kind_, hipStream_t st_ = nullptr, int weight_ = 1, bool enable = true)
       : c(c_), kind(kind_), st(st_ ? st_ : c_->stream), weight(weight_) {
-    on = (c->prof_mask >> kind) & 1u;
+    on = enable && ((c->prof_mask >> kind) & 1u);
     if (on) {
       hipEventCreate(&e0);
       hipEventCreate(&e1);
diff --git a/uncertainty-detection-autolabeling_amd/csrc/uda_internal.h b/uncertainty-detection-autolabeling_amd/csrc/uda_internal.h
--- a/uncertainty-detection-autolabeling_amd/csrc/uda_internal.h
+++ b/uncertainty-detection-autolabeling_amd/csrc/uda_internal.h
@@ -198,6 +198,8 @@
 size_t mbx_par_floats(int Cmid, int k);
 void mbx_pack_params(const float* wd, const float* sc1, const float* sh1, int Cmid, int k, float* out);
 void launch_mbxb(const MbxArgs& a, int rows, int k, int stride, hipStream_t s);
+bool launch_mbx_pw_pair(const MbxArgs& m, int mrows, int k, int stride, const PwArgs& p, int prows, hipStream_t s);
+bool mbx_pw_pair_supported(const MbxArgs& m, int mrows, int k, int stride, const PwArgs& p);
 void launch_mbxd(const MbxArgs& a, int rows, int k, int stride, hipStream_t s);
 bool mbxd_supported(int Cin, int Cmid, int k, int stride);
 size_t mbx_lds_bytes(int Cin, int Cmid, int k, int stride, int scheme, int Ho, int Wo);
diff --git a/uncertainty-detection-autolabeling_amd/plan.py b/uncertainty-detection-autolabeling_amd/plan.py
--- a/uncertainty-detection-autolabeling_amd/plan.py
+++ b/uncertainty-detection-autolabeling_amd/plan.py
@@ -36,7 +36,7 @@
 PW_SCHEME_CODES = {"f32": 0, "bf16x2": 2, "bf16x3": 3, "f16x2": 4, "f16": 5}
 
 PLAN_SWITCHES = {"UDA_DEFER_DROPOUT": 1, "UDA_FUSE_SEP": 1, "UDA_FUSE_PROJ": 1, "UDA_FUSE_MBX": 1, "UDA_FUSE_MBX6": 1,
-                 "UDA_FUSE_MBXD": 1, "UDA_FUSE_IN": 1, "UDA_SEP_MULTI": 1}
+                 "UDA_FUSE_MBXD": 1, "UDA_FUSE_IN": 1, "UDA_SEP_MULTI": 1, "UDA_PAIR_PW": 1}
 
 
 def pw_scheme():
@@ -85,6 +85,21 @@
     if mbx_deep(cin):
         return sch != "f32" and (cin + 1 + 15) // 16 in (6, 8, 13, 14)
     return 16 <= cin
+
+
+def pair_variant(cin, k, stride, sch):
+    return sch in ("f16x2", "bf16x3") and not mbx_deep(cin) and (k, stride, (cin + 1 + 15) // 16) in ((3, 1, 2), (5, 2, 2), (5, 1, 3), (3, 2, 3))
+
+
+PAIR_TABLE = {
+    (3, 1, 24, 144, 96, 24): True,
+    (3, 1, 24, 144, 144, 24): True,
+    (5, 2, 24, 144, 144, 24): True,
+    (5, 2, 24, 144, 144, 40): False,
+    (5, 1, 40, 240, 144, 40): False,
+    (5, 1, 40, 240, 240, 40): False,
+    (3, 2, 40, 240, 240, 40): True,
+}
 
 
 def sepf_supported(C, Cout, sch):
@@ -258,6 +273,9 @@
             return
         self._build_sites()
         self._lower()
+        self.half_windows, self.op_half_win = [], []
+        if sw["UDA_PAIR_PW"] and self.cfg.get("uda_pair_pw", True) and self.chunk_images >= 2:
+            self._mark_half_windows()
         self._plan_memory()
         self.mark_f16_storage()
 
@@ -618,6 +636,57 @@
     def _rows(self, b):
         return self.chunk_images * (self.T if b.per_sample else 1)
 
+    def _mark_half_windows(self):
+        ops, bufs = self.ops, self.bufs
+        hw = self.op_half_win = [0] * len(ops)
+
+        def narrow_pw(o):
+            return (o["kind"] == capi.OP_PW and bufs[o["out"]].C <= 64 and bufs[o["ins"][0]].C < 256 and bufs[o["out"]].kind == 0
+                    and bufs[o["ins"][0]].per_sample == bufs[o["out"]].per_sample)
+
+        def block_after(ip):
+            if ip + 2 >= len(ops):
+                return None
+            m, s = ops[ip + 1], ops[ip + 2]
+            ib, ob = bufs[ops[ip]["out"]], bufs[m["out"]]
+            if not (m["kind"] == capi.OP_MBX and m["ins"] == [ops[ip]["out"]] and m["se_scale"] < 0 and m["se_partial"] >= 0
+                    and ib.per_sample == ob.per_sample and pair_variant(ib.C, m["k"], m["stride"], self.pw_scheme)):
+                return None
+            if not (s["kind"] == capi.OP_SE and s["ins"][0] == m["se_partial"] and bufs[s["out"]].per_sample == ob.per_sample):
+                return None
+            return m, s
+
+        def own_pw(ip):
+            p, m, s = ops[ip], ops[ip - 2], ops[ip - 1]
+            return narrow_pw(p) and p["ins"] == [m["out"]] and p["se_scale"] == s["out"]
+
+        def key(m, p):
+            return (m["k"], m["stride"], bufs[m["ins"][0]].C, bufs[m["out"]].C, bufs[p["ins"][0]].C, bufs[p["out"]].C)
+
+        ip = 0
+        while ip < len(ops):
+            if not (narrow_pw(ops[ip]) and block_after(ip)):
+                ip += 1
+                continue
+            ws, last_p = ip, ip
+            while True:
+                m, _ = block_after(last_p)
+                im = last_p + 1
+                hw[im] = 1 if PAIR_TABLE.get(key(m, ops[last_p])) else 0
+                nxt = last_p + 3
+                if nxt < len(ops) and own_pw(nxt) and block_after(nxt):
+                    hw[im] |= 2 if PAIR_TABLE.get(key(m, ops[nxt])) else 0
+                    last_p = nxt
+                else:
+                    break
+            n = last_p + 3 - ws
+            if any(hw[q] for q in range(ws + 1, ws + n, 3)):
+                hw[ws] = n
+                self.half_windows.append((ws, n))
+            else:
+                hw[ws + 1:ws + n] = [0] * (n - 1)
+            ip = ws + n
+
     def _plan_memory(self):
         for oi, o in enumerate(self.ops):
             touched = list(o["ins"]) + [o["out"]] + [o[k] for k in ("se_scale", "se_partial", "residual") if o[k] >= 0]
@@ -641,6 +710,14 @@
                         buf = self.bufs[b]
                         buf.last = max(buf.last, end)
                         buf.first = min(buf.first, oi)
+        for ws, n in self.half_windows:
+            for ip in range(ws, ws + n, 3):
+                o = self.ops[ip]
+                for b in list(o["ins"]) + [o["out"]] + [o[k] for k in ("se_scale", "residual") if o[k] >= 0]:
+                    buf = self.bufs[b]
+                    buf.last = max(buf.last, ip + 1)
+                    if ip > ws:
+                        buf.first = min(buf.first, ip - 2)
         free, top = [], 0
 
         def alloc(size):
@@ -776,7 +853,8 @@
                 setattr(c, k, int(o[k]))
             c.fuse_in = int(o.get("fuse_in", 0))
             c.fuse_act = int(o.get("fuse_act", 0))
-        sites = (capi.DropSite * max(1, len(self.sites)))()
+            c.half_win = int(self.op_half_win[i]) if self.op_half_win else 0
+        sites =(capi.DropSite * max(1, len(self.sites)))()
         for i, (_, ch, r) in enumerate(self.sites):
             sites[i].channels, sites[i].rate = ch, np.float32(r)
         blob = np.concatenate(self.blob) if self.blob else np.zeros(4, np.float32)
```

New measurement: 5277 (median of 6 runs). No clear change (+0.7%).
